# Shigangli/Ok-Topk

Hardware: NVIDIA H100
Metric: train_samples_per_sec_vgg16_oktopk_density0.001 (higher is better)
Workload: dtype fp32

## Files before the change

oktopk_b200/csrc/bindings.cpp:

```cpp
#include <pybind11/pybind11.h>
#include <pybind11/stl.h>
#include <cuda.h>
#include <cuda_runtime.h>

#include <unistd.h>

#include <algorithm>
#include <cstring>
#include <stdexcept>
#include <string>
#include <tuple>
#include <vector>

#include "oktopk.cuh"

namespace py = pybind11;
using namespace okt;

static void ck(cudaError_t e, const char* what) {
    if (e != cudaSuccess) throw std::runtime_error(std::string(what) + ": " + cudaGetErrorString(e));
}
template <class T> static T* P_(uint64_t p) { return reinterpret_cast<T*>(p); }
static cudaStream_t S_(uint64_t s) { return reinterpret_cast<cudaStream_t>(s); }

// ... 97 lines not shown
}
static uint64_t vmm_import(int fd) {
    auto imp = drv::sym<CUresult (*)(CUmemGenericAllocationHandle*, void*, CUmemAllocationHandleType)>("cuMemImportFromShareableHandle");
    CUmemGenericAllocationHandle h = 0;
    drv::ckd(imp(&h, reinterpret_cast<void*>(static_cast<uintptr_t>(fd)), CU_MEM_HANDLE_TYPE_POSIX_FILE_DESCRIPTOR), "cuMemImportFromShareableHandle");
    return (uint64_t)h;
}
static uint64_t vmm_map(uint64_t handle, size_t nbytes, int dev, size_t align) {
    auto reserve = drv::sym<CUresult (*)(CUdeviceptr*, size_t, size_t, CUdeviceptr, unsigned long long)>("cuMemAddressReserve");
    auto map = drv::sym<CUresult (*)(CUdeviceptr, size_t, size_t, CUmemGenericAllocationHandle, unsigned long long)>("cuMemMap");
    auto access = drv::sym<CUresult (*)(CUdeviceptr, size_t, const CUmemAccessDesc*, size_t)>("cuMemSetAccess");
    CUdeviceptr va = 0;
    drv::ckd(reserve(&va, nbytes, align, 0, 0), "cuMemAddressReserve");
    drv::ckd(map(va, nbytes, 0, (CUmemGenericAllocationHandle)handle, 0), "cuMemMap");
    CUmemAccessDesc ad;
    std::memset(&ad, 0, sizeof(ad));
    ad.location.type = CU_MEM_LOCATION_TYPE_DEVICE;
    ad.location.id = dev;
    ad.flags = CU_MEM_ACCESS_FLAGS_PROT_READWRITE;
    drv::ckd(access(va, nbytes, &ad, 1), "cuMemSetAccess");
    return (uint64_t)va;
}
static void vmm_unmap(uint64_t va, size_t nbytes) {
    auto unmap = drv::sym<CUresult (*)(CUdeviceptr, size_t)>("cuMemUnmap");
    auto afree = drv::sym<CUresult (*)(CUdeviceptr, size_t)>("cuMemAddressFree");
    unmap((CUdeviceptr)va, nbytes);
    afree((CUdeviceptr)va, nbytes);
}
static void vmm_release(uint64_t handle) {
    auto rel = drv::sym<CUresult (*)(CUmemGenericAllocationHandle)>("cuMemRelease");
    rel((CUmemGenericAllocationHandle)handle);
}
static py::tuple mc_create(size_t nbytes, int ndev) {
    auto create = drv::sym<CUresult (*)(CUmemGenericAllocationHandle*, const CUmulticastObjectProp*)>("cuMulticastCreate");
    auto exp = drv::sym<CUresult (*)(void*, CUmemGenericAllocationHandle, CUmemAllocationHandleType, unsigned long long)>("cuMemExportToShareableHandle");
    CUmulticastObjectProp mp;
    std::memset(&mp, 0, sizeof(mp));
    mp.numDevices = ndev; mp.size = nbytes; mp.handleTypes = CU_MEM_HANDLE_TYPE_POSIX_FILE_DESCRIPTOR;
    CUmemGenericAllocationHandle h = 0;
    drv::ckd(create(&h, &mp), "cuMulticastCreate");
    int fd = -1;
    drv::ckd(exp(&fd, h, CU_MEM_HANDLE_TYPE_POSIX_FILE_DESCRIPTOR, 0), "cuMemExportToShareableHandle(mc)");
    return py::make_tuple((uint64_t)h, fd);
}
static void mc_add_device(uint64_t mc, int dev) {
    auto add = drv::sym<CUresult (*)(CUmemGenericAllocationHandle, CUdevice)>("cuMulticastAddDevice");
    drv::ckd(add((CUmemGenericAllocationHandle)mc, dev), "cuMulticastAddDevice");
}
static void mc_bind(uint64_t mc, uint64_t mem, size_t nbytes) {
    auto bind = drv::sym<CUresult (*)(CUmemGenericAllocationHandle, size_t, CUmemGenericAllocationHandle, size_t, size_t, unsigned long long)>("cuMulticastBindMem");
    drv::ckd(bind((CUmemGenericAllocationHandle)mc, 0, (CUmemGenericAllocationHandle)mem, 0, nbytes, 0), "cuMulticastBindMem");
}

static size_t state_bytes() { return sizeof(OktState); }

static py::dict layout_info(int P, int n, int cap, int gcap) {
    SymmLayout L = make_layout(P, n, cap, gcap);
    py::dict d;
    d["total"] = L.total; d["rs_mbox"] = L.rs_mbox; d["rs_thr"] = L.rs_thr; d["ag_mbox"] = L.ag_mbox;
    d["cut_mbox"] = L.cut_mbox; d["cut_data"] = L.cut_data; d["send_idx"] = L.send_idx; d["send_val"] = L.send_val;
    d["gat_idx"] = L.gat_idx; d["gat_val"] = L.gat_val; d["cap"] = L.cap; d["gcap"] = L.gcap; d["scap"] = L.scap;
    d["done_mbox"] = L.done_mbox; d["tree_mbox"] = L.tree_mbox; d["scale_mbox"] = L.scale_mbox;
    d["chunk"] = kChunk; d["maxp"] = OKT_MAXP; d["threads"] = kThreads;
    return d;
}

static py::dict read_state(uint64_t st, int P, uint64_t stream) {
    static thread_local std::vector<char> host(offsetof(OktState, hist));
    ck(cudaMemcpyAsync(host.data(), P_<void>(st), host.size(), cudaMemcpyDeviceToHost, S_(stream)), "read_state");
    ck(cudaStreamSynchronize(S_(stream)), "read_state sync");
    const OktState* s = reinterpret_cast<const OktState*>(host.data());
    py::dict d;
    d["local_thr"] = s->local_thr; d["local_thr_used"] = s->local_thr_used; d["global_thr"] = s->global_thr;
    d["epoch"] = s->epoch;
    std::vector<int> e(s->edges, s->edges + P + 1);
    d["edges"] = e;
    d["local_count"] = s->stat_local_count; d["global_count"] = s->stat_global_count;
    d["recv_total"] = s->stat_recv_total; d["gather_total"] = s->stat_gather_total;
    d["overflow_send"] = s->stat_overflow_send; d["overflow_gather"] = s->stat_overflow_gather;
    d["redo"] = s->stat_redo; d["dense_fallback"] = s->stat_dense_fallback; d["pack_thr"] = s->pack_thr;
    d["cum_overflow_send"] = s->cum_overflow_send; d["cum_overflow_gather"] = s->cum_overflow_gather;
    d["cum_redo"] = s->cum_redo;
    d["fault"] = s->fault;
    auto us = [&](int a, int b) { return s->t_phase[b] >= s->t_phase[a] ? (double)(s->t_phase[b] - s->t_phase[a]) * 1e-3 : 0.0; };
    py::dict ph;
    ph["local"] = us(5, 0); ph["pack"] = us(0, 1); ph["wait_rs"] = us(1, 6); ph["reduce"] = us(6, 2); ph["gselect"] = us(2, 3);
    ph["wait_ag"] = us(3, 7); ph["final"] = us(7, 4); ph["total"] = us(5, 4);
    d["phase_us"] = ph;
    return d;
}

static py::list read_trace(uint64_t st, uint64_t stream) {
    std::vector<TraceRec> host(kTraceLen);
    ck(cudaMemcpyAsync(host.data(), reinterpret_cast<char*>(P_<OktState>(st)) + offsetof(OktState, trace),
                       sizeof(TraceRec) * kTraceLen, cudaMemcpyDeviceToHost, S_(stream)), "read_trace");
    ck(cudaStreamSynchronize(S_(stream)), "read_trace sync");
    py::list out;
    for (const TraceRec& t : host) {
        if (t.epoch == 0) continue;
        py::dict d;
        d["epoch"] = t.epoch; d["local_count"] = t.local_count; d["global_count"] = t.global_count;
        d["recv_total"] = t.recv_total; d["gather_total"] = t.gather_total; d["overflow_send"] = t.overflow_send;
        d["overflow_gather"] = t.overflow_gather; d["redo"] = t.redo; d["local_thr"] = t.local_thr;
        d["global_thr"] = t.global_thr; d["us_local"] = t.us_local; d["us_pack"] = t.us_pack;
        d["us_wait_rs"] = t.us_wait_rs; d["us_reduce"] = t.us_reduce; d["us_gselect"] = t.us_gselect;
        d["us_wait_ag"] = t.us_wait_ag; d["us_final"] = t.us_final; d["t_begin"] = t.t_begin;
        out.append(d);
    }
    return out;
}

static py::tuple host_flag_alloc() {
    int* h = nullptr;
    ck(cudaHostAlloc(reinterpret_cast<void**>(&h), sizeof(int) * 16, cudaHostAllocMapped), "cudaHostAlloc(flag)");
    for (int i = 0; i < 16; ++i) h[i] = 0;
    void* d = nullptr;
    ck(cudaHostGetDevicePointer(&d, h, 0), "cudaHostGetDevicePointer");
    return py::make_tuple((uint64_t)h, (uint64_t)d);
}
static void host_flag_free(uint64_t h) { if (h) cudaFreeHost(P_<void>(h)); }
static int host_flag_read(uint64_t h) { return h ? *reinterpret_cast<volatile int*>(h) : 0; }
static void host_flag_clear(uint64_t h) { if (h) *reinterpret_cast<volatile int*>(h) = 0; }

static void write_state(uint64_t st, float local_thr, float global_thr, const std::vector<int>& edges, uint64_t stream) {
    std::vector<char> host(offsetof(OktState, hist));
    ck(cudaMemcpyAsync(host.data(), P_<void>(st), host.size(), cudaMemcpyDeviceToHost, S_(stream)), "write_state rd");
    ck(cudaStreamSynchronize(S_(stream)), "write_state sync");
    OktState* s = reinterpret_cast<OktState*>(host.data());
    s->local_thr = local_thr;
    s->global_thr = global_thr;
    if (!edges.empty()) {
        if (edges.size() > OKT_MAXP + 1) throw std::runtime_error("too many region edges");
        for (size_t i = 0; i < edges.size(); ++i) s->edges[i] = edges[i];
    }
    ck(cudaMemcpyAsync(P_<void>(st), host.data(), host.size(), cudaMemcpyHostToDevice, S_(stream)), "write_state wr");
    ck(cudaStreamSynchronize(S_(stream)), "write_state sync2");
}

static void fill_peers(char** dst, const std::vector<uint64_t>& peers) {
    if (peers.size() > OKT_MAXP) throw std::runtime_error("world larger than OKT_MAXP");
    for (int i = 0; i < OKT_MAXP; ++i) dst[i] = nullptr;
    for (size_t i = 0; i < peers.size(); ++i) dst[i] = P_<char>(peers[i]);
}

static void oktopk_run(uint64_t g, uint64_t res, uint64_t st, const std::vector<uint64_t>& peers, int n, int rank,
                       int k, int cap, int gcap, py::dict o, int grid, uint64_t stream) {
    OktParams p;
    std::memset(&p, 0, sizeof(p));
    p.g = P_<float>(g); p.res = P_<float>(res); p.st = P_<OktState>(st);
    if (!o.contains("cand") || !o.contains("ccap")) throw std::runtime_error("oktopk_run: candidate scratch missing");
    p.cand = P_<int>(o["cand"].cast<uint64_t>()); p.ccap = o["ccap"].cast<int>();
    p.cand_mode = o.contains("cand_mode") ? o["cand_mode"].cast<int>() : 1;
    fill_peers(p.peers, peers);
    p.P = (int)peers.size(); p.rank = rank; p.n = n; p.k = k;
    p.L = make_layout(p.P, n, cap, gcap);
    auto geti = [&](const char* key, int dflt) { return o.contains(key) ? o[key].cast<int>() : dflt; };
    auto getf = [&](const char* key, double dflt) { return o.contains(key) ? o[key].cast<double>() : dflt; };
    for (int i = 0; i < OKT_MAXP; ++i) p.peer_g[i] = nullptr;
    if (o.contains("peer_g")) {
        auto pg = o["peer_g"].cast<std::vector<uint64_t>>();
        for (size_t i = 0; i < pg.size() && i < OKT_MAXP; ++i) p.peer_g[i] = P_<float>(pg[i]);
    }
    p.max_redo = geti("max_redo", 12);
    p.redo_factor = (float)getf("redo_factor", 1.5);
    p.dense_nnz_limit = geti("dense_nnz_limit", 0);
    p.host_fault = o.contains("host_fault") ? P_<int>(o["host_fault"].cast<uint64_t>()) : nullptr;
    p.skip = o.contains("skip") ? P_<const int>(o["skip"].cast<uint64_t>()) : nullptr;
    p.trace = geti("trace", 0);
    p.exact_local = geti("exact_local", 0);
    p.repartition = geti("repartition", 0);
    p.uniform_regions = geti("uniform_regions", 0);
    p.residual_mode = geti("residual_mode", RES_OKTOPK);
    p.global_mode = geti("global_mode", GLB_THRESHOLD);
    p.deterministic = geti("deterministic", 0);
    p.pull_tma = geti("pull_tma", 1);
    p.phase_begin = geti("phase_begin", 0);
    p.phase_end = geti("phase_end", PH_END);
    p.guard_loops = geti("guard_loops", 0);
    if (p.guard_loops > kGuardFineMax) p.guard_loops = kGuardFineMax;
    p.cap_limit = geti("cap_limit", 0);
    p.cap_rungs = geti("cap_rungs", 40);
    p.cap_factor = (float)getf("cap_factor", 1.19);
    p.guard_limit = geti("guard_limit", 0);
    p.guard_factor = (float)getf("guard_factor", 1.03);
    p.l_low_cnt = getf("l_low_cnt", 0.0); p.l_high_cnt = getf("l_high_cnt", 1e30);
    p.l_factor = (float)getf("l_factor", 1.012);
    p.g_low_cnt = getf("g_low_cnt", 0.0); p.g_high_cnt = getf("g_high_cnt", 1e30);
    p.g_inc = (float)getf("g_inc", 1.008); p.g_dec = (float)getf("g_dec", 1.008);
    p.prefilter = (float)getf("prefilter", 0.8);
    p.timeout_ns = (unsigned long long)(getf("timeout_s", 0.0) * 1e9);
    if (o.contains("srcs")) {
        auto t = o["srcs"].cast<std::tuple<std::vector<uint64_t>, std::vector<long long>, std::vector<long long>>>();
        const auto& ptr = std::get<0>(t);
        const auto& off = std::get<1>(t);
        const auto& len = std::get<2>(t);
        if (off.size() != ptr.size() || len.size() != ptr.size()) throw std::runtime_error("oktopk_run: srcs table size mismatch");
        if (ptr.size() > (size_t)kSrcSegMax) throw std::runtime_error("oktopk_run: more gradient sources than kSrcSegMax");
        long long end = 0;
        for (size_t i = 0; i < ptr.size(); ++i) {
            if (off[i] < end || (off[i] & 3) || len[i] <= 0 || off[i] + len[i] > n || (ptr[i] & 15))
                throw std::runtime_error("oktopk_run: gradient sources must be 16-byte aligned, in bucket order, "
                                         "non-overlapping, at offsets that are multiples of 4 elements");
            p.src[i] = P_<const float>(ptr[i]);
            p.src_off[i] = (int)off[i];
            p.src_len[i] = (int)len[i];
            end = off[i] + len[i];
        }
        p.nsrc = (int)ptr.size();
        p.zero_g = 0;
    } else {
        if (g & 15) throw std::runtime_error("oktopk_run: the bucket must be 16-byte aligned");
        p.src[0] = P_<const float>(g);
        p.src_off[0] = 0;
        p.src_len[0] = n;
        p.nsrc = 1;
        p.zero_g = 1;
    }
    if (o.contains("pack_ranges")) {
        auto rs = o["pack_ranges"].cast<std::vector<std::pair<long long, long long>>>();
        if (rs.size() > (size_t)kPackRangeMax) throw std::runtime_error("oktopk_run: more pack ranges than kPackRangeMax");
        long long end = 0;
        for (size_t i = 0; i < rs.size(); ++i) {
            const long long lo = rs[i].first, hi = rs[i].second;
            if (lo < end || hi < lo || (lo & 3) || (hi & 3) || hi > ((long long)n & ~3LL))
                throw std::runtime_error("oktopk_run: pack ranges must be ordered, disjoint, at multiples of 4 elements, "
                                         "inside the bucket's whole vectors");
            p.pk_lo[i] = (int)(lo >> 2);
            p.pk_hi[i] = (int)(hi >> 2);
            end = hi;
        }
        p.pk_mode = 1;
        p.pk_nr = (int)rs.size();
        if (geti("segment", 0)) {
            if (rs.empty() || p.zero_g || p.L.cap > 0 || p.residual_mode != RES_OKTOPK)
                throw std::runtime_error("oktopk_run: a segment launch takes ranges of an Ok-Topk bucket read from its "
// ... 67 lines not shown
static void land_grads(const std::vector<uint64_t>& srcs, const std::vector<long long>& offs, const std::vector<int>& numels,
                       uint64_t bucket, uint64_t stream) {
    const size_t T = srcs.size();
    if (offs.size() != T || numels.size() != T) throw std::runtime_error("land_grads: table size mismatch");
    constexpr int per = 8192;
    for (size_t b = 0; b < T; b += kLandMax) {
        LandParams lp;
        std::memset(&lp, 0, sizeof(lp));
        const int cnt = (int)std::min<size_t>(kLandMax, T - b);
        int blk = 0;
        for (int i = 0; i < cnt; ++i) {
            lp.src[i] = P_<const float>(srcs[b + i]);
            lp.dst_off[i] = offs[b + i];
            lp.numel[i] = numels[b + i];
            lp.blk_begin[i] = blk;
            blk += std::max(1, (numels[b + i] + per - 1) / per);
        }
        lp.blk_begin[cnt] = blk;
        lp.count = cnt;
        ck(launch_land(lp, P_<float>(bucket), S_(stream)), "land_grads");
    }
}

static void dense_run(const std::vector<uint64_t>& bufs, const std::vector<uint64_t>& flags, uint64_t epoch, int n,
                      int rank, int grid, uint64_t stream, uint64_t st, double timeout_s, uint64_t mc,
                      uint64_t host_fault, uint64_t skip) {
    DenseParams p;
    std::memset(&p, 0, sizeof(p));
    if (bufs.size() > OKT_MAXP || bufs.size() != flags.size()) throw std::runtime_error("bad peer tables");
    for (size_t i = 0; i < bufs.size(); ++i) { p.bufs[i] = P_<float>(bufs[i]); p.flags[i] = P_<uint64_t>(flags[i]); }
    p.epoch = P_<unsigned long long>(epoch);
    p.n = n; p.P = (int)bufs.size(); p.rank = rank; p.scale = 1.0f / (float)p.P;
    p.fault = st ? &P_<OktState>(st)->fault : nullptr;
    p.timeout_ns = (unsigned long long)(timeout_s * 1e9);
    p.mc = P_<float>(mc);
    p.host_fault = P_<int>(host_fault);
    p.skip = P_<const int>(skip);
    ck(launch_dense_allreduce(p, grid, S_(stream)), "dense allreduce launch");
}

static void kth_abs(uint64_t x, int n, int k, uint64_t st, uint64_t out, int grid, uint64_t stream) {
    ck(launch_kth_abs(P_<float>(x), n, k, P_<OktState>(st), P_<float>(out), grid, S_(stream)), "kth_abs launch");
}

static void fused_sgd(uint64_t p, uint64_t g, uint64_t mom, int n, double momentum, double dampening, double wd,
                      int nesterov, int first, int zero_grad, uint64_t stream, uint64_t scal_ptr, uint64_t fault_ptr,
                      uint64_t skip_ptr, uint64_t coef_ptr) {
    if (scal_ptr == 0) throw std::runtime_error("fused_sgd: scal_ptr must point at the group's device scalars");
    ck(launch_fused_sgd(P_<float>(p), P_<float>(g), P_<float>(mom), n, (float)momentum, (float)dampening, (float)wd,
                        nesterov, first, zero_grad, P_<float>(scal_ptr), P_<int>(fault_ptr), P_<int>(skip_ptr),
                        P_<const float>(coef_ptr), S_(stream)),
       "fused_sgd");
}
static SgdRanges sgd_ranges(const std::vector<std::pair<long long, long long>>& rs, int n, const char* what) {
    if ((int)rs.size() > kPackRangeMax)
        throw std::runtime_error(std::string(what) + ": more than " + std::to_string(kPackRangeMax) + " ranges");
    SgdRanges r;
    std::memset(&r, 0, sizeof(r));
    r.nr = (int)rs.size();
    for (int q = 0; q < r.nr; ++q) {
        const long long lo = rs[q].first, hi = rs[q].second;
        if (lo < 0 || hi < lo || lo % 4 || hi % 4 || hi > 4LL * (n / 4))
            throw std::runtime_error(std::string(what) + ": ranges must lie at multiples of 4 inside the slice's whole "
                                     "float4 vectors");
        r.lo[q] = (int)(lo / 4);
        r.hi[q] = (int)(hi / 4);
    }
    return r;
}
static void sgd_ahead(uint64_t p, uint64_t mom, uint64_t sp, uint64_t sm, int n,
                      const std::vector<std::pair<long long, long long>>& ranges, double momentum, double dampening,
                      double wd, int nesterov, int max_ctas, uint64_t stream, uint64_t scal_ptr) {
    if (scal_ptr == 0) throw std::runtime_error("sgd_ahead: scal_ptr must point at the group's device scalars");
    if (momentum != 0.0 && (mom == 0 || sm == 0)) throw std::runtime_error("sgd_ahead: momentum needs mom and sm");
    const SgdHyper h{(float)momentum, (float)dampening, (float)wd, nesterov, 0};
    ck(launch_sgd_ahead(P_<float>(p), P_<float>(mom), P_<float>(sp), P_<float>(sm), sgd_ranges(ranges, n, "sgd_ahead"),
                        h, max_ctas, P_<float>(scal_ptr), S_(stream)),
       "sgd_ahead");
}
static void fused_sgd_tail(uint64_t p, uint64_t g, uint64_t mom, uint64_t sp, uint64_t sm, int n,
                           const std::vector<std::pair<long long, long long>>& ahead,
                           const std::vector<std::pair<long long, long long>>& dense, double momentum, double dampening,
                           double wd, int nesterov, int first, int zero_grad, uint64_t stream, uint64_t scal_ptr,
                           uint64_t fault_ptr, uint64_t skip_ptr, uint64_t coef_ptr) {
    if (scal_ptr == 0) throw std::runtime_error("fused_sgd_tail: scal_ptr must point at the group's device scalars");
    if (momentum != 0.0 && (mom == 0 || sm == 0)) throw std::runtime_error("fused_sgd_tail: momentum needs mom and sm");
    const SgdHyper h{(float)momentum, (float)dampening, (float)wd, nesterov, first};
    ck(launch_fused_sgd_tail(P_<float>(p), P_<float>(g), P_<float>(mom), P_<const float>(sp), P_<const float>(sm), n,
                             sgd_ranges(ahead, n, "fused_sgd_tail"), sgd_ranges(dense, n, "fused_sgd_tail"), h,
                             zero_grad, P_<float>(scal_ptr), P_<int>(fault_ptr), P_<int>(skip_ptr),
                             P_<const float>(coef_ptr), S_(stream)),
       "fused_sgd_tail");
}
static void fused_bert_adam(uint64_t p, uint64_t g, uint64_t m, uint64_t v, int n, double b1, double b2, double eps,
                            double wd, int zero_grad, uint64_t stream, uint64_t scal_ptr, uint64_t fault_ptr,
                            uint64_t skip_ptr, uint64_t coef_ptr, uint64_t ends_ptr) {
    if (scal_ptr == 0) throw std::runtime_error("fused_bert_adam: scal_ptr must point at the group's device scalars");
    if (ends_ptr != 0 && coef_ptr == 0) throw std::runtime_error("fused_bert_adam: segment ends need the factors");
    const ClipRef clip{P_<const float>(coef_ptr), P_<const int>(ends_ptr)};
    ck(launch_fused_bert_adam(P_<float>(p), P_<float>(g), P_<float>(m), P_<float>(v), n, (float)b1, (float)b2,
                              (float)eps, (float)wd, zero_grad, P_<float>(scal_ptr), P_<int>(fault_ptr), P_<int>(skip_ptr),
                              clip, S_(stream)),
       "fused_bert_adam");
}
static void fused_adam(uint64_t p, uint64_t g, uint64_t m, uint64_t v, int n, double beta1, double beta2, double eps,
                       double wd, int decoupled, int zero_grad, uint64_t stream, uint64_t scal_ptr, uint64_t fault_ptr,
                       uint64_t skip_ptr, uint64_t coef_ptr) {
    if (scal_ptr == 0) throw std::runtime_error("fused_adam: scal_ptr must point at the group's device scalars");
    ck(launch_fused_adam(P_<float>(p), P_<float>(g), P_<float>(m), P_<float>(v), n, beta1, beta2, (float)eps, (float)wd,
                         decoupled, zero_grad, P_<float>(scal_ptr), P_<int>(fault_ptr), P_<int>(skip_ptr),
                         P_<const float>(coef_ptr), S_(stream)),
       "fused_adam");
}
static void fused_lamb(uint64_t p, uint64_t g, uint64_t m, uint64_t v, int n, double beta1, double beta2, double eps,
                       int nseg, uint64_t off, uint64_t len, uint64_t blk, uint64_t ends, int nblk, uint64_t part_w,
                       uint64_t part_u, uint64_t norm_w, uint64_t norm_u, uint64_t ratio, int zero_grad,
                       uint64_t stream, uint64_t scal_ptr, uint64_t fault_ptr, uint64_t skip_ptr, uint64_t coef_ptr) {
    if (scal_ptr == 0) throw std::runtime_error("fused_lamb: scal_ptr must point at the group's device scalars");
    if (nseg <= 0 || nblk < nseg || n < 0 || !off || !len || !blk || !ends || !part_w || !part_u || !norm_w || !norm_u ||
        !ratio)
        throw std::runtime_error("fused_lamb: bad segment table or buffers");
    if ((p | g | m | v) % 16 || (part_w | part_u) % 8)
        throw std::runtime_error("fused_lamb: p, g, m and v must be 16-byte aligned");
    const LambSegs t{P_<const int>(off), P_<const int>(len), P_<const int>(blk), P_<const int>(ends), nseg};
    ck(launch_fused_lamb(P_<float>(p), P_<float>(g), P_<float>(m), P_<float>(v), n, beta1, beta2, (float)eps, t, nblk,
                         P_<double>(part_w), P_<double>(part_u), P_<float>(norm_w), P_<float>(norm_u), P_<float>(ratio),
                         zero_grad, P_<float>(scal_ptr), P_<int>(fault_ptr), P_<int>(skip_ptr),
                         P_<const float>(coef_ptr), S_(stream)),
       "fused_lamb");
}
static Dtype dtype_arg(int dtype, const char* what) {
    if (dtype < 0 || dtype > 2) throw std::runtime_error(std::string(what) + ": dtype must be 0 (fp32), 1 (bf16) or 2 (fp16)");
    return static_cast<Dtype>(dtype);
}
static void bn_forward(uint64_t x, uint64_t y, uint64_t arg, uint64_t partial, uint64_t gamma, uint64_t beta, uint64_t cbias,
                       uint64_t save_mean, uint64_t save_invstd, uint64_t rmean, uint64_t rvar, uint64_t nbt, double momentum,
                       double eps, int relu, int M, int C, int W, int slot, int max_ctas, uint64_t stream, int dtype,
                       uint64_t res) {
    if (C % 4 != 0) throw std::runtime_error("bn_forward: channel count must be a multiple of 4");
    if (slot < 0) throw std::runtime_error("bn_forward: negative slot");
    if (res != 0 && (W != 0 || !relu)) throw std::runtime_error("bn_forward: a residual needs relu = 1 and no pool");
    ck(launch_bn_forward(P_<const void>(x), P_<void>(y), P_<unsigned char>(arg), P_<float>(partial), P_<const float>(gamma),
                         P_<const float>(beta), P_<const float>(cbias), P_<float>(save_mean), P_<float>(save_invstd),
                         P_<float>(rmean), P_<float>(rvar), P_<long long>(nbt), (float)momentum, (float)eps, relu, M, C, W, slot,
                         max_ctas, dtype_arg(dtype, "bn_forward"), S_(stream), P_<const void>(res)), "bn_forward");
}
static void bn_backward(uint64_t x, uint64_t dy, uint64_t arg, uint64_t dx, uint64_t partial, uint64_t gamma, uint64_t beta,
                        uint64_t save_mean, uint64_t save_invstd, uint64_t dgamma, uint64_t dbeta, int relu, int M, int C, int W,
                        int slot, int max_ctas, uint64_t stream, int dtype, uint64_t res, uint64_t dres) {
    if (slot < 0) throw std::runtime_error("bn_backward: negative slot");
    if ((res == 0) != (dres == 0)) throw std::runtime_error("bn_backward: res and dres go together");
    if (res != 0 && (W != 0 || !relu)) throw std::runtime_error("bn_backward: a residual needs relu = 1 and no pool");
    ck(launch_bn_backward(P_<const void>(x), P_<const void>(dy), P_<const unsigned char>(arg), P_<void>(dx), P_<float>(partial),
                          P_<const float>(gamma), P_<const float>(beta), P_<const float>(save_mean), P_<const float>(save_invstd),
                          P_<float>(dgamma), P_<float>(dbeta), relu, M, C, W, slot, max_ctas, dtype_arg(dtype, "bn_backward"),
                          S_(stream), P_<const void>(res), P_<void>(dres)), "bn_backward");
}
static void ln_check(const char* what, int R, int H, long long p_keep_thr, uint64_t seed, uint64_t mean, uint64_t rstd,
                     std::initializer_list<uint64_t> vec_ptrs) {
    if (R <= 0 || !ln_supported_h(H)) throw std::runtime_error(std::string(what) + ": needs R > 0 and H in 128, 256, ..., 1024");
    if (p_keep_thr < 0 || p_keep_thr > (1LL << 32)) throw std::runtime_error(std::string(what) + ": p_keep_thr out of range");
    if (p_keep_thr < (1LL << 32) && seed == 0) throw std::runtime_error(std::string(what) + ": dropout needs the seed");
    if (mean == 0 || rstd == 0) throw std::runtime_error(std::string(what) + ": mean and rstd are needed");
    for (uint64_t p : vec_ptrs)
        if (p == 0 || (p & 15)) throw std::runtime_error(std::string(what) + ": tensors must be non-null and 16-byte aligned");
}
static void ln_forward(uint64_t x, uint64_t a, uint64_t y, uint64_t gamma, uint64_t beta, uint64_t mean, uint64_t rstd,
                       uint64_t seed, int R, int H, long long p_keep_thr, double scale, double eps, int a_dtype,
                       uint64_t stream) {
    ln_check("ln_forward", R, H, p_keep_thr, seed, mean, rstd, {x, a, y, gamma, beta});
    ck(launch_ln_forward(P_<const float>(x), P_<const void>(a), P_<float>(y), P_<const float>(gamma), P_<const float>(beta),
                         P_<float>(mean), P_<float>(rstd), P_<const unsigned long long>(seed), R, H, p_keep_thr, (float)scale,
                         (float)eps, dtype_arg(a_dtype, "ln_forward"), S_(stream)), "ln_forward");
}
// ... 261 lines not shown
        t.nseg = (int)std::min<size_t>(kSrcSegMax, T - b);
        long long blk = 0;
        for (int i = 0; i < t.nseg; ++i) {
            const long long o = offs[b + i], l = lens[b + i];
            if (o < 0 || o % 4 || l < 0 || o + l > (1LL << 31) - 1)
                throw std::runtime_error("grad_sumsq: segments must lie at multiples of 4 inside an int32 range");
            t.off[i] = (int)o;
            t.len[i] = (int)l;
            t.blk_begin[i] = (int)blk;
            blk += std::max(1LL, (l + kSumsqChunk - 1) / kSumsqChunk);
        }
        t.blk_begin[t.nseg] = (int)blk;
        ck(launch_grad_sumsq(P_<const float>(g), t, out, S_(stream)), "grad_sumsq");
        out += blk;
    }
}
static void clip_coef(uint64_t partial, int np, uint64_t seg_blk, uint64_t seg_scal, int nseg, uint64_t scal,
                      double max_norm, uint64_t norm, uint64_t coef, uint64_t stream) {
    if (seg_blk != 0 && (seg_scal == 0 || scal == 0 || nseg <= 0))
        throw std::runtime_error("clip_coef: per-segment factors need seg_scal, scal and nseg");
    ck(launch_clip_coef(P_<const double>(partial), np, P_<const int>(seg_blk), P_<const int>(seg_scal), nseg,
                        P_<const float>(scal), (float)max_norm, P_<float>(norm), P_<float>(coef), S_(stream)),
       "clip_coef");
}

static void unscale_check(const std::vector<uint64_t>& srcs, const std::vector<long long>& lens, uint64_t ls, uint64_t sync,
                          uint64_t st, uint64_t host_fault, const std::vector<uint64_t>& peers, size_t mbox_off, int rank,
                          double timeout_s, uint64_t stream) {
    ScaleParams p;
    std::memset(&p, 0, sizeof(p));
    if (srcs.empty() || srcs.size() != lens.size()) throw std::runtime_error("unscale_check: bad source table");
    if (srcs.size() > (size_t)kSrcSegMax) throw std::runtime_error("unscale_check: more gradient sources than kSrcSegMax");
    if (peers.size() > OKT_MAXP) throw std::runtime_error("world larger than OKT_MAXP");
    int blk = 0;
    for (size_t i = 0; i < srcs.size(); ++i) {
        if ((srcs[i] & 15) || lens[i] <= 0 || lens[i] > (1LL << 31) - 1)
            throw std::runtime_error("unscale_check: sources must be 16-byte aligned and non-empty");
        p.src[i] = P_<float>(srcs[i]);
        p.len[i] = (int)lens[i];
        p.blk_begin[i] = blk;
        blk += (int)((lens[i] + kScalePerCta - 1) / kScalePerCta);
    }
    p.blk_begin[srcs.size()] = blk;
    p.nseg = (int)srcs.size();
    p.ls = P_<LossScaleDev>(ls);
    p.sync = P_<ScaleSync>(sync);
    p.fault = &P_<OktState>(st)->fault;
    p.host_fault = P_<int>(host_fault);
    for (size_t i = 0; i < peers.size(); ++i) p.peers[i] = P_<char>(peers[i]);
    p.mbox_off = mbox_off;
    p.P = (int)peers.size(); p.rank = rank;
    p.timeout_ns = (unsigned long long)(timeout_s * 1e9);
    ck(launch_unscale_check(p, S_(stream)), "unscale_check");
}

PYBIND11_MODULE(_C, m) {
    m.doc() = "oktopk_b200 native extension (sm_90a kernels + symmetric peer memory)";
    m.def("symm_alloc", &symm_alloc);
    m.def("symm_open", &symm_open);
    m.def("symm_close", &symm_close);
    m.def("symm_free", &symm_free);
    m.def("dev_alloc_zero", &dev_alloc_zero);
    m.def("dev_free", &dev_free);
    m.def("memset_async", &memset_async);
    m.def("can_access_peer", &can_access_peer);
    m.def("state_bytes", &state_bytes);
    m.def("layout_info", &layout_info);
    m.def("read_state", &read_state);
    m.def("write_state", &write_state);
    m.def("max_coop_grid", &okt_max_coop_grid);
    m.def("oktopk_run", &oktopk_run);
    m.def("gather_run", &gather_run);
    m.def("dense_run", &dense_run, py::arg("bufs"), py::arg("flags"), py::arg("epoch"), py::arg("n"), py::arg("rank"),
          py::arg("grid"), py::arg("stream"), py::arg("st") = 0, py::arg("timeout_s") = 0.0, py::arg("mc") = 0,
          py::arg("host_fault") = 0, py::arg("skip") = 0);
    m.def("gtopk_run", &gtopk_run);
    m.def("land_grads", &land_grads);
    m.def("read_trace", &read_trace);
    m.def("host_flag_alloc", &host_flag_alloc);
    m.def("host_flag_free", &host_flag_free);
    m.def("host_flag_read", &host_flag_read);
    m.def("host_flag_clear", &host_flag_clear);
    m.def("fault_ptr", [](uint64_t st) { return (uint64_t)&P_<OktState>(st)->fault; });
    m.def("gather_max_coop_grid", &gather_max_coop_grid);
    m.def("gtopk_max_coop_grid", &gtopk_max_coop_grid);
    m.def("vmm_probe", &vmm_probe);
    m.def("vmm_create", &vmm_create);
    m.def("vmm_import", &vmm_import);
    m.def("vmm_map", &vmm_map);
    m.def("vmm_unmap", &vmm_unmap);
    m.def("vmm_release", &vmm_release);
    m.def("mc_create", &mc_create);
    m.def("mc_add_device", &mc_add_device);
    m.def("mc_bind", &mc_bind);
    m.def("close_fd", [](int fd) { if (fd >= 0) ::close(fd); });
    m.def("clear_fault", [](uint64_t st, uint64_t stream) {
        ck(cudaMemsetAsync(&P_<OktState>(st)->fault, 0, sizeof(int), S_(stream)), "clear_fault");
    });
    m.def("kth_abs", &kth_abs);
    m.def("fused_sgd", &fused_sgd, py::arg("p"), py::arg("g"), py::arg("mom"), py::arg("n"), py::arg("momentum"),
          py::arg("dampening"), py::arg("wd"), py::arg("nesterov"), py::arg("first"), py::arg("zero_grad"),
          py::arg("stream"), py::arg("scal_ptr"), py::arg("fault_ptr") = 0, py::arg("skip_ptr") = 0,
          py::arg("coef_ptr") = 0);
    m.def("sgd_ahead", &sgd_ahead, py::arg("p"), py::arg("mom"), py::arg("sp"), py::arg("sm"), py::arg("n"),
          py::arg("ranges"), py::arg("momentum"), py::arg("dampening"), py::arg("wd"), py::arg("nesterov"),
          py::arg("max_ctas"), py::arg("stream"), py::arg("scal_ptr"));
    m.def("fused_sgd_tail", &fused_sgd_tail, py::arg("p"), py::arg("g"), py::arg("mom"), py::arg("sp"), py::arg("sm"),
          py::arg("n"), py::arg("ahead"), py::arg("dense"), py::arg("momentum"), py::arg("dampening"), py::arg("wd"),
          py::arg("nesterov"), py::arg("first"), py::arg("zero_grad"), py::arg("stream"), py::arg("scal_ptr"),
          py::arg("fault_ptr") = 0, py::arg("skip_ptr") = 0, py::arg("coef_ptr") = 0);
    m.def("fused_bert_adam", &fused_bert_adam, py::arg("p"), py::arg("g"), py::arg("m"), py::arg("v"), py::arg("n"),
          py::arg("b1"), py::arg("b2"), py::arg("eps"), py::arg("wd"), py::arg("zero_grad"), py::arg("stream"),
          py::arg("scal_ptr"), py::arg("fault_ptr") = 0, py::arg("skip_ptr") = 0, py::arg("coef_ptr") = 0,
          py::arg("ends_ptr") = 0);
    m.def("fused_adam", &fused_adam, py::arg("p"), py::arg("g"), py::arg("m"), py::arg("v"), py::arg("n"),
          py::arg("beta1"), py::arg("beta2"), py::arg("eps"), py::arg("wd"), py::arg("decoupled"), py::arg("zero_grad"),
          py::arg("stream"), py::arg("scal_ptr"), py::arg("fault_ptr") = 0, py::arg("skip_ptr") = 0,
          py::arg("coef_ptr") = 0);
    m.def("fused_lamb", &fused_lamb, py::arg("p"), py::arg("g"), py::arg("m"), py::arg("v"), py::arg("n"),
          py::arg("beta1"), py::arg("beta2"), py::arg("eps"), py::arg("nseg"), py::arg("off"), py::arg("len"),
          py::arg("blk"), py::arg("ends"), py::arg("nblk"), py::arg("part_w"), py::arg("part_u"), py::arg("norm_w"),
          py::arg("norm_u"), py::arg("ratio"), py::arg("zero_grad"), py::arg("stream"), py::arg("scal_ptr"),
          py::arg("fault_ptr") = 0, py::arg("skip_ptr") = 0, py::arg("coef_ptr") = 0);
    m.def("momentum_correct", &momentum_correct);
    m.def("grad_sumsq", &grad_sumsq, py::arg("g"), py::arg("offs"), py::arg("lens"), py::arg("partial"),
          py::arg("stream"));
    m.def("clip_coef", &clip_coef, py::arg("partial"), py::arg("np"), py::arg("seg_blk"), py::arg("seg_scal"),
          py::arg("nseg"), py::arg("scal"), py::arg("max_norm"), py::arg("norm"), py::arg("coef"), py::arg("stream"));
    m.def("unscale_check", &unscale_check);
    m.def("scale_update", [](uint64_t ls, double growth, double backoff, int interval, uint64_t stream) {
        ck(launch_scale_update(P_<LossScaleDev>(ls), growth, backoff, interval, S_(stream)), "scale_update");
    });
    m.def("adam_scalars", [](uint64_t ls, uint64_t hyper, uint64_t scal, int groups, uint64_t stream, int lamb) {
        ck(launch_adam_scalars(P_<const LossScaleDev>(ls), P_<const double>(hyper), P_<float>(scal), groups, lamb,
                               S_(stream)),
           "adam_scalars");
    }, py::arg("ls"), py::arg("hyper"), py::arg("scal"), py::arg("groups"), py::arg("stream"), py::arg("lamb") = 0);
    m.def("carry_residual", [](uint64_t g, uint64_t res, int n, uint64_t skip, uint64_t stream) {
        ck(launch_carry_residual(P_<float>(g), P_<float>(res), n, P_<const int>(skip), S_(stream)), "carry_residual");
    });
    m.attr("LOSS_SCALE_BYTES") = sizeof(LossScaleDev);
    m.attr("SCALE_SYNC_BYTES") = sizeof(ScaleSync);
    m.attr("VERDICT_OFFSET") = offsetof(ScaleSync, verdict);
    m.def("maxpool2_fwd", &maxpool2_fwd);
    m.def("maxpool2_bwd", &maxpool2_bwd);
    m.def("bn_forward", &bn_forward, py::arg("x"), py::arg("y"), py::arg("arg"), py::arg("partial"), py::arg("gamma"),
          py::arg("beta"), py::arg("cbias"), py::arg("save_mean"), py::arg("save_invstd"), py::arg("rmean"), py::arg("rvar"),
          py::arg("nbt"), py::arg("momentum"), py::arg("eps"), py::arg("relu"), py::arg("M"), py::arg("C"), py::arg("W"),
          py::arg("slot"), py::arg("max_ctas"), py::arg("stream"), py::arg("dtype"), py::arg("res") = 0);
    m.def("bn_backward", &bn_backward, py::arg("x"), py::arg("dy"), py::arg("arg"), py::arg("dx"), py::arg("partial"),
          py::arg("gamma"), py::arg("beta"), py::arg("save_mean"), py::arg("save_invstd"), py::arg("dgamma"), py::arg("dbeta"),
          py::arg("relu"), py::arg("M"), py::arg("C"), py::arg("W"), py::arg("slot"), py::arg("max_ctas"), py::arg("stream"),
          py::arg("dtype"), py::arg("res") = 0, py::arg("dres") = 0);
    m.def("bn_tile_rows", &bn_tile_rows);
    m.def("bn_sliced", &bn_sliced, py::arg("M"), py::arg("C"), py::arg("W"));
    m.def("ln_forward", &ln_forward, py::arg("x"), py::arg("a"), py::arg("y"), py::arg("gamma"), py::arg("beta"),
          py::arg("mean"), py::arg("rstd"), py::arg("seed"), py::arg("R"), py::arg("H"), py::arg("p_keep_thr"),
          py::arg("scale"), py::arg("eps"), py::arg("a_dtype"), py::arg("stream"));
    m.def("ln_backward", &ln_backward, py::arg("x"), py::arg("a"), py::arg("dy"), py::arg("gamma"), py::arg("mean"),
          py::arg("rstd"), py::arg("seed"), py::arg("dx"), py::arg("da"), py::arg("partial"), py::arg("dgamma"),
          py::arg("dbeta"), py::arg("R"), py::arg("H"), py::arg("p_keep_thr"), py::arg("scale"), py::arg("a_dtype"),
          py::arg("stream"));
    m.def("ln_bwd_grid", &ln_bwd_grid);
    m.def("ln_supported_h", &ln_supported_h);
    m.def("emb_forward", &emb_forward, py::arg("ids"), py::arg("tt"), py::arg("word"), py::arg("pos"), py::arg("typ"),
          py::arg("gamma"), py::arg("beta"), py::arg("y"), py::arg("stats"), py::arg("ovf"), py::arg("seed"), py::arg("R"),
          py::arg("S"), py::arg("H"), py::arg("nv"), py::arg("np"), py::arg("nt"), py::arg("p_keep_thr"), py::arg("scale"),
          py::arg("eps"), py::arg("stream"));
    m.def("emb_backward", &emb_backward, py::arg("ids"), py::arg("tt"), py::arg("word"), py::arg("pos"), py::arg("typ"),
          py::arg("gamma"), py::arg("stats"), py::arg("dy"), py::arg("seed"), py::arg("de"), py::arg("partial"), py::arg("dgamma"), py::arg("dbeta"), py::arg("dword"), py::arg("dpos"), py::arg("dtyp"),
          py::arg("R"), py::arg("S"), py::arg("H"), py::arg("nv"), py::arg("np"), py::arg("nt"), py::arg("p_keep_thr"),
          py::arg("scale"), py::arg("stream"));
    m.def("emb_supported", &emb_supported);
    m.def("attn_forward", &attn_forward, py::arg("qkv"), py::arg("mask"), py::arg("seed"), py::arg("out"), py::arg("lse"),
          py::arg("B"), py::arg("S"), py::arg("H"), py::arg("p_keep_thr"), py::arg("scale"), py::arg("dtype"),
          py::arg("stream"));
    m.def("attn_backward", &attn_backward, py::arg("qkv"), py::arg("out"), py::arg("dout"), py::arg("mask"), py::arg("seed"),
          py::arg("lse"), py::arg("delta"), py::arg("dqkv"), py::arg("B"), py::arg("S"), py::arg("H"), py::arg("p_keep_thr"),
          py::arg("scale"), py::arg("dtype"), py::arg("stream"));
    m.def("attn_supported", &attn_supported);
    m.def("xent_forward", &xent_forward, py::arg("x"), py::arg("t"), py::arg("lse"), py::arg("rowloss"), py::arg("loss"),
          py::arg("R"), py::arg("V"), py::arg("ignore_index"), py::arg("dtype"), py::arg("stream"));
    m.def("xent_backward", &xent_backward, py::arg("x"), py::arg("t"), py::arg("lse"), py::arg("g"), py::arg("dx"),
          py::arg("R"), py::arg("V"), py::arg("ignore_index"), py::arg("dtype"), py::arg("stream"));
    m.def("ctc_forward", &ctc_forward, py::arg("x"), py::arg("t"), py::arg("t64"), py::arg("tn"), py::arg("ln"),
          py::arg("ws"), py::arg("loss"), py::arg("T"), py::arg("N"), py::arg("C"), py::arg("nt"), py::arg("dtype"),
          py::arg("stream"));
    m.def("ctc_backward", &ctc_backward, py::arg("x"), py::arg("t"), py::arg("t64"), py::arg("tn"), py::arg("ln"),
          py::arg("ws"), py::arg("ab"), py::arg("g"), py::arg("dx"), py::arg("T"), py::arg("N"), py::arg("C"), py::arg("nt"),
          py::arg("dtype"), py::arg("stream"));
    m.def("ctc_supported", &ctc_supported);
    m.def("frame_bn_forward", &frame_bn_forward, py::arg("conv"), py::arg("x"), py::arg("len"), py::arg("gamma"),
          py::arg("beta"), py::arg("y"), py::arg("mean"), py::arg("rstd"), py::arg("rmean"), py::arg("rvar"),
// ... 43 lines not shown
```

oktopk_b200/csrc/oktopk.cu:

```cuda
#include "devlib.cuh"

namespace okt {

__device__ __forceinline__ int region_of(const int* s_edges, int P, int i) {
    int d = 0;
#pragma unroll 1
    for (int r = 1; r < P; ++r) d += (i >= s_edges[r]) ? 1 : 0;
    return d;
}

struct SrcSeg { const float* src; int off, len; };

__device__ __forceinline__ int seg_find(const SrcSeg* s, int ns, int e) {
    int lo = 0, hi = ns - 1, r = -1;
    while (lo <= hi) {
        const int mid = (lo + hi) >> 1;
        if (s[mid].off <= e) { r = mid; lo = mid + 1; } else { hi = mid - 1; }
    }
    return r;
}

__device__ __forceinline__ float grad_at(const SrcSeg* s, int ns, int i) {
    const int q = seg_find(s, ns, i);
    return (q >= 0 && i - s[q].off < s[q].len) ? s[q].src[i - s[q].off] : 0.f;
// ... 200 lines not shown
                const int lo_d = sel.edges[d], hi_d = sel.edges[d + 1];
                mine = 0u;
#pragma unroll
                for (int u = 0; u < kPackTile; ++u) {
#pragma unroll
                    for (int c = 0; c < 4; ++c) {
                        const int i = 4 * (base + u * kThreads + tid) + c;
                        const bool pd = ((mybits >> (u * 4 + c)) & 1u) && i >= lo_d && i < hi_d;
                        md[u * 4 + c] = __ballot_sync(0xffffffffu, pd);
                        cnt += __popc(md[u * 4 + c]);
                        if (pd) mine |= 1u << (u * 4 + c);
                    }
                }
            }
            if (cnt == 0) continue;
            int run = 0;
            if (lane == 0) run = atomicAdd(&st->send_cursor[d], cnt);
            run = __shfl_sync(0xffffffffu, run, 0);
            const int scap_d = sel.soff[d + 1] - sel.soff[d];
            int* sidx = sel.sidx + sel.soff[d];
            float* sval = sel.sval + sel.soff[d];
            const int off_d = sel.edges[d];
            const unsigned lt = (1u << lane) - 1u;
#pragma unroll
            for (int u = 0; u < kPackTile; ++u) {
                const float xs[4] = {a[u].x, a[u].y, a[u].z, a[u].w};
#pragma unroll
                for (int c = 0; c < 4; ++c) {
                    const int q = u * 4 + c;
                    if ((mine >> q) & 1u) {
                        const int pos = run + __popc(md[q] & lt);
                        const int i = 4 * (base + u * kThreads + tid) + c;
                        if (pos < scap_d) {
                            sidx[pos] = i - off_d;
                            sval[pos] = xs[c];
                            if (p.residual_mode != RES_OKTOPK) p.res[i] = 0.f;
                        } else {
                            dropped++;
                        }
                    }
                    run += __popc(md[q]);
                }
            }
        }
    }
    return nmine;
}

__global__ void __launch_bounds__(kThreads, kCtasPerSm) oktopk_fused_kernel(const OktParams p) {
    __shared__ uint32_t s_hist[kHistBins];
    __shared__ int s_w[kWarps + 1];
    __shared__ int s_edges[OKT_MAXP + 1];
    __shared__ int s_cnt[OKT_MAXP];
    __shared__ float s_thr[OKT_MAXP];
    __shared__ int s_misc[OKT_MAXP * 2 + 4];
    __shared__ int s_soff[OKT_MAXP + 1];
    __shared__ float s_lthr[kGuardMax];
    __shared__ int s_lcnt[kGuardMax];
    __shared__ ChunkSrc s_srcs[OKT_MAXP];
    __shared__ float s_sthr[OKT_MAXP];
    __shared__ Seg s_segs[OKT_MAXP];
    __shared__ __align__(128) PullSmem s_pull;
    __shared__ __align__(8) uint64_t s_pk_bar[kPackStages];
    __shared__ __align__(8) uint64_t s_pk_empty[kPackStages];
    __shared__ __align__(8) uint64_t s_sc_bar[kScanStages];
    __shared__ SrcSeg s_src[kSrcSegMax];
    __shared__ int s_tail_v[kSrcSegMax], s_tail_q[kSrcSegMax];
    __shared__ int s_ntail;
    __shared__ int s_rlo[kPackRangeMax], s_rhi[kPackRangeMax], s_rfirst[kPackRangeMax + 1];
    extern __shared__ __align__(128) float4 dyn_pk[];

    if (verdict_set(p.skip)) return;
    OktState* st = p.st;
    const int tid = threadIdx.x, lane = tid & 31, warp = tid >> 5;
    const int gtid = blockIdx.x * kThreads + tid;
    const int gthreads = gridDim.x * kThreads;
    const int P = p.P, rank = p.rank, n = p.n;
    char* me = p.peers[rank];
    const uint32_t epoch = st->epoch + 1u;
    const int par = epoch & 1u;
    const float thr_in = st->local_thr;
    const bool exact_local = p.exact_local || thr_in == 0.f;
    const bool two_pass = exact_local || p.repartition;
    uint32_t pipe_it = 0;

    for (int b = tid; b < kHistBins; b += kThreads) s_hist[b] = 0;
    if (blockIdx.x == 0 && tid == 0) st->t_phase[5] = globaltimer_ns();
    const SpinGuard sg_rs{&st->fault, p.timeout_ns, FAULT_RS_TIMEOUT, p.host_fault};
    const SpinGuard sg_ag{&st->fault, p.timeout_ns, FAULT_AG_TIMEOUT, p.host_fault};
    const SpinGuard sg_cut{&st->fault, p.timeout_ns, FAULT_CUT_TIMEOUT, p.host_fault};
    const SpinGuard sg_done{&st->fault, p.timeout_ns, FAULT_DONE_TIMEOUT, p.host_fault};
    if (tid == 0) {
        mbar_init(&s_pull.bar[0], 1);
        mbar_init(&s_pull.bar[1], 1);
        for (int q = 0; q < kPackStages; ++q) { mbar_init(&s_pk_bar[q], 1); mbar_init(&s_pk_empty[q], kWarps); }
        for (int q = 0; q < kScanStages; ++q) mbar_init(&s_sc_bar[q], 1);
        mbar_fence_init();
    }
    const int n4 = n >> 2;
    const int nsrc = p.nsrc;
    load_src_table(p, s_src, s_tail_v, s_tail_q, &s_ntail);
    const int ntail = s_ntail;
    const int whole[2] = {0, n4};
    const bool ranged = p.pk_mode && !two_pass;
    const TileMap tmap = tile_map_build(ranged ? p.pk_nr : 1, ranged ? p.pk_lo : whole, ranged ? p.pk_hi : whole + 1,
                                        s_rlo, s_rhi, s_rfirst);

    float4* r4 = reinterpret_cast<float4*>(p.res);

    if (p.phase_begin <= PH_LOCAL && PH_LOCAL < p.phase_end && two_pass) {
        const float thr0 = thr_in;
        const LadderCfg lcl = ladder_cfg(p, !exact_local);
        ladder_build(s_lthr, s_lcnt, lcl, thr0);

        auto visit = [&](float x) {
            if (exact_local) {
                hist_add(s_hist, x, 0, 0u);
            } else {
                float ax = fabsf(x);
                if (ax > thr0) atomicAdd(&s_lcnt[ladder_rung(s_lthr, lcl.n_total, ax)], 1);
            }
        };
        const float cut = (exact_local && thr0 > 0.f) ? thr0 * p.prefilter : -1.f;
        const bool prefilter = cut > 0.f;
        constexpr int kLocTile = 4;
        for (int base = blockIdx.x * kThreads * kLocTile; base < n4; base += gridDim.x * kThreads * kLocTile) {
            float4 a[kLocTile], r[kLocTile];
            bool in[kLocTile];
#pragma unroll
            for (int u = 0; u < kLocTile; ++u) {
                const int v = base + u * kThreads + tid;
                in[u] = v < n4;
                if (in[u]) { a[u] = grad4_at(s_src, nsrc, v); r[u] = ld_stream_f4(r4 + v); }
                else { a[u] = make_float4(0.f, 0.f, 0.f, 0.f); r[u] = a[u]; }
            }
#pragma unroll
            for (int u = 0; u < kLocTile; ++u) {
                const int v = base + u * kThreads + tid;
                a[u].x += r[u].x; a[u].y += r[u].y; a[u].z += r[u].z; a[u].w += r[u].w;
                if (in[u]) st_stream_f4(r4 + v, a[u]);
                const float xs[4] = {a[u].x, a[u].y, a[u].z, a[u].w};
                if (!prefilter) {
                    if (in[u]) { visit(xs[0]); visit(xs[1]); visit(xs[2]); visit(xs[3]); }
                    continue;
                }
                unsigned bits = 0u;
                int tot = 0;
#pragma unroll
                for (int c = 0; c < 4; ++c) {
                    const bool pd = in[u] && fabsf(xs[c]) > cut;
                    if (pd) bits |= 1u << c;
                    tot += __popc(__ballot_sync(0xffffffffu, pd));
                }
                if (tot == 0) continue;
                int run = 0;
                if (lane == 0) run = atomicAdd(&st->cand_cursor, tot);
                run = __shfl_sync(0xffffffffu, run, 0);
#pragma unroll
                for (int c = 0; c < 4; ++c) {
                    const bool pd = (bits >> c) & 1u;
                    const unsigned m = __ballot_sync(0xffffffffu, pd);
                    if (pd) {
                        const int pos = run + __popc(m & ((1u << lane) - 1u));
                        if (pos < p.ccap) p.cand[pos] = 4 * v + c;
                    }
                    run += __popc(m);
// ... 165 lines not shown
            auto emit = [&](int i, float x, bool inrange) {
                const float ax = fabsf(x);
                const bool pred = inrange && ax > thr_sel;
                unsigned todo = __ballot_sync(0xffffffffu, pred);
                if (todo == 0) return;
                int d = 0;
                if (pred) {
                    d = region_of(s_edges, P, i);
                    atomicAdd(&s_lcnt[lc.n_total > 1 ? ladder_rung(s_lthr, lc.n_total, ax) : 0], 1);
                }
                while (todo) {
                    const int leader = __ffs(todo) - 1;
                    const int dl = __shfl_sync(0xffffffffu, d, leader);
                    const bool mine = pred && d == dl;
                    const unsigned m = __ballot_sync(0xffffffffu, mine);
                    int base = 0;
                    if (lane == leader) base = atomicAdd(&st->send_cursor[dl], __popc(m));
                    base = __shfl_sync(0xffffffffu, base, leader);
                    if (mine) {
                        const int pos = base + __popc(m & ((1u << lane) - 1u));
                        if (pos < s_soff[dl + 1] - s_soff[dl]) {
                            my_sidx[s_soff[dl] + pos] = i - s_edges[dl];
                            my_sval[s_soff[dl] + pos] = x;
                            if (p.residual_mode != RES_OKTOPK) p.res[i] = 0.f;
                        } else {
                            dropped++;
                        }
                    }
                    todo &= ~m;
                }
            };

            const PackSrc src{s_src, nsrc, s_tail_v, s_tail_q, ntail};
            const PackSel sel{thr_sel, lc, s_lthr, s_lcnt, s_edges, s_soff, my_sidx, my_sval, P};
            ring_it += pack_stream<kPackStages>(p, tmap, ring, ring_it, res_only, attempt == 0 && p.zero_g, src, sel, dropped);
            if (blockIdx.x == 0 && warp == 0 && (n & 3)) {
                int i = n4 * 4 + lane;
                bool in = i < n;
                float a = 0.f;
                if (in) {
                    a = res_only ? p.res[i] : (grad_at(s_src, nsrc, i) + p.res[i]);
                    if (!res_only) p.res[i] = a;
                    if (p.zero_g) p.g[i] = 0.f;
                }
                emit(i, a, in);
            }
            if (p.residual_mode == RES_LOCAL_GE && blockIdx.x == 0 && (n & 3)) {
                for (int i = n4 * 4 + tid; i < n; i += kThreads) {
                    float x = p.res[i];
                    if (x != 0.f && fabsf(x) == thr_sel && atomicAdd(&st->tie_cursor, 1) < (int)__ldcg(&st->sel_krem))
                        p.res[i] = 0.f;
                }
            }
            ladder_flush(st, s_lcnt);
            if (!can_redo) break;
            grid_sync(&st->bar);
            bool over = false;
            for (int d = 0; d < P; ++d) over = over || (__ldcg(&st->send_cursor[d]) > s_soff[d + 1] - s_soff[d]);
            if (!over || attempt >= p.max_redo) break;
            grid_sync(&st->bar);
            if (blockIdx.x == 0 && tid == 0) {
                for (int d = 0; d < P; ++d) st->send_cursor[d] = 0;
                for (int q = 0; q < kGuardMax; ++q) st->guard_counts[q] = 0;
                st->cum_redo += 1ULL;
            }
            thr_sel = fmaxf(thr_sel, 1e-30f) * redo_f;
            redo_f = fminf(redo_f * redo_f, 1e6f);
            ++attempt;
            grid_sync(&st->bar);
        }
        {
            int dsum = warp_sum(dropped);
            if (lane == 0 && dsum) atomicAdd(&st->cum_overflow_send, (unsigned long long)dsum);
        }
        const bool publisher = can_redo ? (blockIdx.x == 0) : last_cta_ticket(&st->tick[0]);
        if (publisher) {
            if (tid == 0) {
                int cnt;
                const float t = ladder_pick(st, ladder_cfg(p, !two_pass), thr_sel, p.guard_limit, p.cap_limit, &cnt);
                st->local_thr_used = t;
                st->pack_thr = thr_sel;
                st->stat_local_count = cnt;
                st->tie_cursor = 0;
                float nt = t;
                if ((double)cnt < p.l_low_cnt) nt = t / p.l_factor;
                else if ((double)cnt > p.l_high_cnt) nt = t * p.l_factor;
                st->local_thr = nt;
                s_thr[0] = t;
                __threadfence();
            }
            __syncthreads();
            if (tid < P) {
                const int c = min(__ldcg(&st->send_cursor[tid]), s_soff[tid + 1] - s_soff[tid]);
                st_relaxed_sys_u32(reinterpret_cast<uint32_t*>(rs_thr(p.peers[tid], p.L, par, rank)), __float_as_uint(s_thr[0]));
                st_release_sys_u64(rs_mbox(p.peers[tid], p.L, par, rank), make_mail(epoch, (uint32_t)c));
            }
            __syncthreads();
        }
        stamp(1);
    }

    if (p.phase_begin <= PH_REDUCE && PH_REDUCE < p.phase_end) {
        if (tid < P) {
            s_cnt[tid] = (int)wait_mailbox(rs_mbox(me, p.L, par, tid), epoch, sg_rs);
            s_thr[tid] = __uint_as_float(ld_relaxed_sys_u32(reinterpret_cast<uint32_t*>(rs_thr(me, p.L, par, tid))));
        }
        __syncthreads();
        stamp(6);
        const int off_me = s_edges[rank];
        const int len_me = s_edges[rank + 1] - off_me;
        float* greg = p.g + off_me;
        int pulled = 0;
        auto add = [&](int s_local, int idx, float val, const float* thr_of) {
            const bool ok = fabsf(val) > thr_of[s_local] && (unsigned)idx < (unsigned)len_me;
            if (p.cand_mode) {
                float old = 1.f;
                if (ok) old = atomicAdd(greg + idx, val);
                const bool first = ok && old == 0.f;
                const int pos = warp_append_active(&st->cand_cursor, first);
                if (first && pos < p.ccap) p.cand[pos] = idx;
            } else if (ok) {
                red_add_f32(greg + idx, val);
            }
            pulled++;
        };
        const int my_soff = s_soff[rank];
        if (!p.deterministic) {
            if (tid < P) {
                const int s = (rank + tid) % P;
                s_srcs[tid].idx = send_idx_base(p.peers[s], p.L) + my_soff;
                s_srcs[tid].val = send_val_base(p.peers[s], p.L) + my_soff;
                s_srcs[tid].count = s_cnt[s];
                s_sthr[tid] = s_thr[s];
            }
            __syncthreads();
            pull_chunks(s_srcs, P, p.pull_tma != 0, &s_pull, pipe_it,
                        [&](int sl, int idx, float val) { add(sl, idx, val, s_sthr); });
        } else {
            for (int s = 0; s < P; ++s) {
                ChunkSrc src{send_idx_base(p.peers[s], p.L) + my_soff, send_val_base(p.peers[s], p.L) + my_soff, s_cnt[s]};
                float thr1 = s_thr[s];
                pull_chunks(&src, 1, p.pull_tma != 0, &s_pull, pipe_it,
                            [&](int, int idx, float val) { add(0, idx, val, &thr1); });
                grid_sync(&st->bar);
            }
        }
        int psum = warp_sum(pulled);
        if (lane == 0 && psum) atomicAdd(&st->stat_recv_total, psum);
        if (PH_REDUCE + 1 < p.phase_end) grid_sync(&st->bar);
        stamp(2);
    }

    if (p.phase_begin <= PH_GSELECT && PH_GSELECT < p.phase_end) {
        const float gthr = st->global_thr;
        const int lo = s_edges[rank], hi = s_edges[rank + 1];
        const int gcap = p.L.gcap;
        int* gi = gat_idx(me, p.L, par);
        float* gv = gat_val(me, p.L, par);
        const bool keep_in_place = p.global_mode == GLB_ALL_NONZERO;
        int dropped = 0;
        if (p.cand_mode) {
            const int ncand = min(*reinterpret_cast<volatile int*>(&st->cand_cursor), p.ccap);
            const int ncr = (ncand + 31) / 32 * 32;
            for (int c = gtid; c < ncr; c += gthreads) {
                const bool in = c < ncand;
                const int i = in ? __ldcg(p.cand + c) : 0;
// ... 71 lines not shown
                        run += __popc(m);
                    }
                    if (!keep_in_place) {
                        if ((nzbits >> (u * 4)) & 0xfu)
                            *reinterpret_cast<float4*>(p.g + first + 4 * (q0 + u * kThreads + tid)) = make_float4(0.f, 0.f, 0.f, 0.f);
                    } else if ((lostbits >> (u * 4)) & 0xfu) {
#pragma unroll
                        for (int c = 0; c < 4; ++c)
                            if ((lostbits >> (u * 4 + c)) & 1u) p.g[first + 4 * (q0 + u * kThreads + tid) + c] = 0.f;
                    }
                }
            });
        }
        int dsum = warp_sum(dropped);
        if (lane == 0 && dsum) atomicAdd(&st->cum_overflow_gather, (unsigned long long)dsum);
        stamp(3);
        if (last_cta_ticket(&st->tick[1])) {
            if (tid == 0) s_misc[0] = min(__ldcg(&st->gather_cursor), p.L.gcap);
            __syncthreads();
            if (tid < P) st_release_sys_u64(ag_mbox(p.peers[tid], p.L, par, rank), make_mail(epoch, (uint32_t)s_misc[0]));
            __syncthreads();
        }
    }

    if (p.phase_begin <= PH_FINAL && PH_FINAL < p.phase_end) {
        if (tid < P) s_cnt[tid] = (int)wait_mailbox(ag_mbox(me, p.L, par, tid), epoch, sg_ag);
        __syncthreads();
        stamp(7);
        int T = 0;
        for (int s = 0; s < P; ++s) T += s_cnt[s];
        const float fP = (float)P;
        const bool dense_path = p.global_mode == GLB_ALL_NONZERO && p.dense_nnz_limit > 0 && T >= p.dense_nnz_limit &&
                                P > 1 && p.peer_g[0] != nullptr;
        int kept_cnt = 0;
        if (dense_path) {
            const float inv = 1.f / fP;
            for (int t = 1; t < P; ++t) {
                const int s = (rank + t) % P;
                const int lo_s = s_edges[s], hi_s = s_edges[s + 1];
                const float* src = p.peer_g[s];
                const int first = min(hi_s, (lo_s + 3) & ~3), last = max(first, hi_s & ~3);
                for (int i = lo_s + gtid; i < first; i += gthreads) p.g[i] = ld_peer_f32(src + i) * inv;
                for (int i = last + gtid; i < hi_s; i += gthreads) p.g[i] = ld_peer_f32(src + i) * inv;
                const int nv = (last - first) >> 2;
                const int4* s4 = reinterpret_cast<const int4*>(src + first);
                float4* d4 = reinterpret_cast<float4*>(p.g + first);
                for (int v = gtid; v < nv; v += gthreads) {
                    const int4 r = ld_peer_i4(s4 + v);
                    st_stream_f4(d4 + v, make_float4(__int_as_float(r.x) * inv, __int_as_float(r.y) * inv,
                                                     __int_as_float(r.z) * inv, __int_as_float(r.w) * inv));
                }
            }
            grid_sync(&st->bar);
            if (blockIdx.x == 0 && tid < P) st_release_sys_u64(done_mbox(p.peers[tid], p.L, par, rank), make_mail(epoch, 1u));
            if (tid < P) wait_mailbox(done_mbox(me, p.L, par, tid), epoch, sg_done);
            __syncthreads();
            const int lo = s_edges[rank], hi = s_edges[rank + 1];
            for (int i = lo + gtid; i < hi; i += gthreads) p.g[i] = __ldcg(p.g + i) * inv;
            if (blockIdx.x == 0 && tid == 0) { st->stat_dense_fallback = 1; st->stat_global_count = T; }
        } else {
            float gsel = 0.f;
            if (p.global_mode == GLB_EXACT_TOPK) {
                if (tid < P) { s_segs[tid].ptr = gat_val(p.peers[tid], p.L, par); s_segs[tid].count = s_cnt[tid]; s_segs[tid].idx = nullptr; }
                __syncthreads();
                const uint32_t kk = (uint32_t)min(T, p.k);
                gsel = (kk > 0) ? grid_kth_abs(s_segs, P, true, kk, st, s_hist, s_w, 0) : 0.f;
                if (blockIdx.x == 0 && tid == 0) st->global_thr = gsel;
            } else if (p.global_mode == GLB_THRESHOLD && blockIdx.x == 0 && tid == 0) {
                float gt = st->global_thr;
                if ((double)T < p.g_low_cnt) gt = gt / p.g_inc;
                else if ((double)T > p.g_high_cnt) gt = gt * p.g_dec;
                st->global_thr = gt;
            }
            const float thr_used = st->local_thr_used;
            if (tid < P) {
                const int s = (rank + tid) % P;
                s_srcs[tid].idx = gat_idx(p.peers[s], p.L, par);
                s_srcs[tid].val = gat_val(p.peers[s], p.L, par);
                s_srcs[tid].count = s_cnt[s];
            }
            __syncthreads();
            const bool exact = p.global_mode == GLB_EXACT_TOPK;
            pull_chunks(s_srcs, P, p.pull_tma != 0, &s_pull, pipe_it, [&](int sl, int idx, float val) {
                if ((unsigned)idx >= (unsigned)n) return;
                bool keep = exact ? (fabsf(val) >= gsel) : true;
                if (!keep) return;
                kept_cnt++;
                p.g[idx] = val / fP;
                if (p.residual_mode == RES_OKTOPK) {
                    float r = p.res[idx];
                    if (fabsf(r) > thr_used) p.res[idx] = 0.f;
                }
            });
            int ksum = warp_sum(kept_cnt);
            if (lane == 0 && ksum) atomicAdd(&st->stat_global_count, ksum);
        }
        if (last_cta_ticket(&st->tick[2]) && tid == 0) {
            const unsigned long long t_end = globaltimer_ns();
            st->epoch = epoch;
            st->t_phase[4] = t_end;
            st->stat_gather_total = T;
            for (int d = 0; d < P; ++d) st->send_cursor[d] = 0;
            st->gather_cursor = 0;
            st->cand_cursor = 0;
            const unsigned long long os = *reinterpret_cast<volatile unsigned long long*>(&st->cum_overflow_send);
            const unsigned long long og = *reinterpret_cast<volatile unsigned long long*>(&st->cum_overflow_gather);
            const unsigned long long rd = *reinterpret_cast<volatile unsigned long long*>(&st->cum_redo);
            st->stat_overflow_send = (int)min(os - st->snap_overflow_send, 0x7fffffffULL);
            st->stat_overflow_gather = (int)min(og - st->snap_overflow_gather, 0x7fffffffULL);
            st->stat_redo = (int)(rd - st->snap_redo);
            st->snap_overflow_send = os; st->snap_overflow_gather = og; st->snap_redo = rd;
            TraceRec& tr = st->trace[epoch % kTraceLen];
            auto us = [&](int a, int b) {
                const unsigned long long ta = *reinterpret_cast<volatile unsigned long long*>(&st->t_phase[a]);
                const unsigned long long tb = *reinterpret_cast<volatile unsigned long long*>(&st->t_phase[b]);
                return tb >= ta ? (float)(tb - ta) * 1e-3f : 0.f;
            };
            tr.epoch = epoch;
            tr.local_count = st->stat_local_count;
            tr.global_count = *reinterpret_cast<volatile int*>(&st->stat_global_count);
            tr.recv_total = *reinterpret_cast<volatile int*>(&st->stat_recv_total);
            tr.gather_total = T;
            tr.overflow_send = st->stat_overflow_send;
            tr.overflow_gather = st->stat_overflow_gather;
            tr.redo = st->stat_redo;
            tr.local_thr = st->local_thr_used;
            tr.global_thr = st->global_thr;
            tr.us_local = us(5, 0); tr.us_pack = us(0, 1); tr.us_wait_rs = us(1, 6); tr.us_reduce = us(6, 2);
            tr.us_gselect = us(2, 3); tr.us_wait_ag = us(3, 7); tr.us_final = us(7, 4);
            tr.t_begin = st->t_phase[5];
        }
    }
}

__global__ void __launch_bounds__(kThreads) oktopk_segment_kernel(const OktParams p) {
    __shared__ int s_edges[OKT_MAXP + 1];
    __shared__ int s_soff[OKT_MAXP + 1];
    __shared__ float s_lthr[kGuardMax];
    __shared__ int s_lcnt[kGuardMax];
    __shared__ __align__(8) uint64_t s_full[kSegStages];
    __shared__ __align__(8) uint64_t s_empty[kSegStages];
    __shared__ SrcSeg s_src[kSrcSegMax];
    __shared__ int s_tail_v[kSrcSegMax], s_tail_q[kSrcSegMax];
    __shared__ int s_ntail;
    __shared__ int s_rlo[kPackRangeMax], s_rhi[kPackRangeMax], s_rfirst[kPackRangeMax + 1];
    extern __shared__ __align__(128) float4 dyn_seg[];

    if (verdict_set(p.skip)) return;
    OktState* st = p.st;
    const float thr = st->local_thr;
    if (thr == 0.f) return;
    const int tid = threadIdx.x, P = p.P;
    if (tid == 0) {
        for (int q = 0; q < kSegStages; ++q) { mbar_init(&s_full[q], 1); mbar_init(&s_empty[q], kWarps); }
        mbar_fence_init();
    }
    if (tid <= P) s_edges[tid] = st->edges[tid];
    load_src_table(p, s_src, s_tail_v, s_tail_q, &s_ntail);
    if (tid <= P) s_soff[tid] = (tid < P) ? slot_off(p.L, s_edges, tid) : slot_off(p.L, s_edges, P);
    const TileMap tmap = tile_map_build(p.pk_nr, p.pk_lo, p.pk_hi, s_rlo, s_rhi, s_rfirst);
    const LadderCfg lc = ladder_cfg(p, true);
    ladder_build(s_lthr, s_lcnt, lc, thr);
    char* me = p.peers[p.rank];
    const PackRing ring{dyn_seg, dyn_seg + kSegStages * kTileV, s_full, s_empty};
    const PackSrc src{s_src, p.nsrc, s_tail_v, s_tail_q, s_ntail};
    const PackSel sel{thr, lc, s_lthr, s_lcnt, s_edges, s_soff, send_idx_base(me, p.L), send_val_base(me, p.L), P};
    int dropped = 0;
    pack_stream<kSegStages>(p, tmap, ring, 0, false, false, src, sel, dropped);
// ... 61 lines not shown
```

oktopk_b200/csrc/oktopk.cuh:

```cuda
#pragma once
#include <cuda_runtime.h>
#include <stdint.h>
#include <stddef.h>

#ifndef OKT_MAXP
#define OKT_MAXP 16
#endif

namespace okt {

constexpr int kThreads = 512;
constexpr int kWarps = kThreads / 32;
constexpr int kChunk = 1024;
constexpr int kHistBins = 2048;
constexpr int kMaxWarpsTotal = 16384;
constexpr int kGuardMax = 64;
constexpr int kGuardFineMax = 15;
constexpr int kCtasPerSm = 1;
constexpr int kPackTile = 2;
constexpr int kPackStages = 4;
constexpr int kPackSmemBytes = kPackStages * 2 * kPackTile * kThreads * 16;
constexpr int kScanStages = 2 * kPackStages;
constexpr int kStrideGridMax = 132 * 8;

constexpr int kTraceLen = 256;
struct TraceRec {
    uint32_t epoch;
    int local_count, global_count, recv_total, gather_total, overflow_send, overflow_gather, redo;
    float local_thr, global_thr;
    float us_local, us_pack, us_wait_rs, us_reduce, us_gselect, us_wait_ag, us_final;
    unsigned long long t_begin;
};

struct OktState {
    unsigned long long bar;
    unsigned int tick[4];
    float local_thr;
    float local_thr_used;
    float global_thr;
    uint32_t epoch;
    int edges[OKT_MAXP + 1];
    int send_cursor[OKT_MAXP];
    int gather_cursor;
    int cand_cursor;
    int guard_counts[kGuardMax];
    uint32_t sel_prefix;
    uint32_t sel_krem;
    int tie_cursor;
    int cuts[OKT_MAXP];
    int stat_local_count;
    int stat_global_count;
    int stat_recv_total;
    int stat_gather_total;
    int stat_overflow_send;
    int stat_overflow_gather;
    int stat_redo;
    int stat_dense_fallback;
    int stat_mode;
    int fault;
    float pack_thr;
    unsigned long long cum_overflow_send;
    unsigned long long cum_overflow_gather;
    unsigned long long cum_redo;
    unsigned long long snap_overflow_send;
    unsigned long long snap_overflow_gather;
    unsigned long long snap_redo;
    unsigned long long t_phase[8];
    double gs_sum, gs_sumsq;
    double clip_sumsq;
    uint32_t hist[kHistBins];
    int wcounts[kMaxWarpsTotal];
    TraceRec trace[kTraceLen];
};

struct SymmLayout {
    size_t rs_mbox;
    size_t rs_thr;
    size_t ag_mbox;
    size_t cut_mbox;
    size_t cut_data;
    size_t done_mbox;
    size_t tree_mbox;
    size_t scale_mbox;
    size_t send_idx;
    size_t send_val;
    size_t gat_idx;
    size_t gat_val;
    size_t total;
    int cap;
    int scap;
    int gcap;
};

inline size_t align_up(size_t x, size_t a) { return (x + a - 1) / a * a; }

inline SymmLayout make_layout(int P, int n, int cap, int gcap) {
    SymmLayout L;
    size_t o = 0;
    L.rs_mbox = o;  o += sizeof(uint64_t) * 2 * OKT_MAXP;
    L.rs_thr = o;   o += sizeof(float) * 2 * OKT_MAXP;
    L.ag_mbox = o;  o += sizeof(uint64_t) * 2 * OKT_MAXP;
    L.cut_mbox = o; o += sizeof(uint64_t) * 2 * OKT_MAXP;
    L.cut_data = o; o += sizeof(int) * 2 * OKT_MAXP * OKT_MAXP;
    L.done_mbox = o; o += sizeof(uint64_t) * 2 * OKT_MAXP;
    L.tree_mbox = o; o += sizeof(uint64_t) * 2 * OKT_MAXP;
    L.scale_mbox = o; o += sizeof(uint64_t) * 2 * OKT_MAXP;
    o = align_up(o, 1024);
    const size_t scap = cap > 0 ? (size_t)P * cap : align_up((size_t)n, 4) + 4 * (size_t)OKT_MAXP + 1024;
    L.send_idx = o; o += sizeof(int) * scap;   o = align_up(o, 1024);
    L.send_val = o; o += sizeof(float) * scap; o = align_up(o, 1024);
    L.gat_idx = o;  o += sizeof(int) * 2 * (size_t)gcap;      o = align_up(o, 1024);
    L.gat_val = o;  o += sizeof(float) * 2 * (size_t)gcap;    o = align_up(o, 1024);
    L.total = o;
    L.cap = cap;
    L.scap = (int)scap;
    L.gcap = gcap;
    return L;
}

enum Phase : int {
    PH_LOCAL = 0,
    PH_PACK = 1,
    PH_PUBLISH_RS = 2,
    PH_REDUCE = 3,
    PH_GSELECT = 4,
    PH_PUBLISH_AG = 5,
    PH_FINAL = 6,
    PH_END = 7
};

enum ResidualMode : int { RES_OKTOPK = 0, RES_LOCAL_GT = 1, RES_LOCAL_GE = 2 };
enum GlobalMode : int { GLB_THRESHOLD = 0, GLB_EXACT_TOPK = 1, GLB_ALL_NONZERO = 2 };

constexpr int kSrcSegMax = 160;
constexpr int kPackRangeMax = 32;
constexpr int kSegStages = 2;
constexpr int kSegTiles = 4;

struct OktParams {
    float* g;
    float* res;
    OktState* st;
    int* cand;
    int ccap;
    int cand_mode;
    float prefilter;
    char* peers[OKT_MAXP];
    float* peer_g[OKT_MAXP];
    SymmLayout L;
    int n, P, rank, k;
    int exact_local, repartition, uniform_regions;
    int residual_mode, global_mode;
    int deterministic, pull_tma;
    int phase_begin, phase_end;
    int guard_loops, guard_limit;
    float guard_factor;
    int cap_limit, cap_rungs;
    float cap_factor;
    double l_low_cnt, l_high_cnt;
    float l_factor;
    double g_low_cnt, g_high_cnt;
    float g_inc, g_dec;
    unsigned long long timeout_ns;
    int max_redo;
    float redo_factor;
    int dense_nnz_limit;
    int* host_fault;
    const int* skip;
    int trace;
    int zero_g;
    int nsrc;
    int src_off[kSrcSegMax];
    int src_len[kSrcSegMax];
    const float* src[kSrcSegMax];
    int pk_mode, pk_nr;
    int pk_lo[kPackRangeMax];
    int pk_hi[kPackRangeMax];
};
static_assert(sizeof(OktParams) <= 4096, "OktParams must fit the 4 KB kernel-parameter limit");

enum GatherSelect : int { GS_THRESHOLD_REUSE = 0, GS_GAUSSIAN = 1, GS_EXACT_TOPK = 2 };

struct GatherParams {
    float* g;
    float* res;
    OktState* st;
    char* peers[OKT_MAXP];
    SymmLayout L;
    int n, P, rank, k;
    int select_mode;
    int exact_now;
    int gauss_mode;
    int gauss_loops;
    float gauss_factor;
    float density;
    int pull_tma;
    unsigned long long timeout_ns;
    int reselect;
    float clip_max_norm;
    unsigned* bitmap;
    int* cand;
    int ccap;
    int* host_fault;
    const int* skip;
};

struct TreeParams {
    float* g;
    float* res;
    OktState* st;
    char* peers[OKT_MAXP];
    SymmLayout L;
    int n, P, rank, k;
    int pull_tma;
    unsigned long long timeout_ns;
    float clip_max_norm;
    unsigned* bitmap;
    int* cand;
    int ccap;
    int* sel_idx;
    float* sel_val;
    int selcap;
    int* host_fault;
    const int* skip;
};

struct DenseParams {
    float* bufs[OKT_MAXP];
    uint64_t* flags[OKT_MAXP];
    unsigned long long* epoch;
    int n, P, rank;
    float scale;
    int* fault;
    unsigned long long timeout_ns;
    float* mc;
    int* host_fault;
    const int* skip;
};

int okt_max_coop_grid(int device);
cudaError_t launch_oktopk(const OktParams& p, int grid, cudaStream_t stream);
cudaError_t launch_oktopk_segment(const OktParams& p, int max_ctas, cudaStream_t stream);
cudaError_t launch_gather_scheme(const GatherParams& p, int grid, cudaStream_t stream);
cudaError_t launch_gtopk(const TreeParams& p, int grid, cudaStream_t stream);
int gtopk_max_coop_grid(int device);
int gather_max_coop_grid(int device);
cudaError_t launch_dense_allreduce(const DenseParams& p, int grid, cudaStream_t stream);
cudaError_t launch_kth_abs(const float* x, int n, int k, OktState* st, float* out_thr, int grid, cudaStream_t stream);
constexpr int kSumsqChunk = 16384;
struct SumsqSegs {
    int nseg;
    int off[kSrcSegMax];
    int len[kSrcSegMax];
    int blk_begin[kSrcSegMax + 1];
};
static_assert(sizeof(SumsqSegs) <= 4096, "SumsqSegs must fit the 4 KB kernel-parameter limit");
cudaError_t launch_grad_sumsq(const float* g, const SumsqSegs& t, double* partial, cudaStream_t stream);
cudaError_t launch_clip_coef(const double* partial, int np, const int* seg_blk, const int* seg_scal, int nseg,
                             const float* scal, float max_norm, float* norm, float* coef, cudaStream_t stream);
struct ClipRef {
    const float* coef;
    const int* ends;
};
cudaError_t launch_fused_sgd(float* p, float* g, float* mom, int n, float momentum, float dampening, float weight_decay,
                             int nesterov, int first_step, int zero_grad, const float* scal, const int* fault,
                             const int* skip, const float* coef, cudaStream_t stream);
struct SgdRanges {
    int nr;
    int lo[kPackRangeMax];
    int hi[kPackRangeMax];
};
struct SgdHyper {
    float momentum, dampening, wd;
    int nesterov, first;
};
cudaError_t launch_sgd_ahead(float* p, float* mom, float* sp, float* sm, const SgdRanges& r, const SgdHyper& h,
                             int max_ctas, const float* scal, cudaStream_t stream);
cudaError_t launch_fused_sgd_tail(float* p, float* g, float* mom, const float* sp, const float* sm, int n,
                                  const SgdRanges& ahead, const SgdRanges& dense, const SgdHyper& h, int zero_grad,
                                  const float* scal, const int* fault, const int* skip, const float* coef,
                                  cudaStream_t stream);
cudaError_t launch_fused_bert_adam(float* p, float* g, float* m, float* v, int n, float b1, float b2, float eps,
                                   float weight_decay, int zero_grad, const float* scal, const int* fault,
                                   const int* skip, const ClipRef& clip, cudaStream_t stream);
cudaError_t launch_fused_adam(float* p, float* g, float* m, float* v, int n, double beta1, double beta2, float eps,
                              float weight_decay, int decoupled, int zero_grad, const float* scal, const int* fault,
                              const int* skip, const float* coef, cudaStream_t stream);
struct LambSegs {
    const int* off;
    const int* len;
    const int* blk;
    const int* ends;
    int nseg;
};
struct LambHyper {
    float b1, omb1, b2, omb2, eps;
};
cudaError_t launch_fused_lamb(float* p, float* g, float* m, float* v, int n, double beta1, double beta2, float eps,
                              const LambSegs& t, int nblk, double* part_w, double* part_u, float* norm_w,
                              float* norm_u, float* ratio, int zero_grad, const float* scal, const int* fault,
                              const int* skip, const float* coef, cudaStream_t stream);

struct LossScaleDev {
    float scale;
    float inv_scale;
    int growth_tracker;
    int found_inf;
    long long skipped;
    long long adam_step;
};
struct ScaleSync {
    int flag;
    unsigned int ticket;
    unsigned int epoch;
    int verdict;
};
constexpr int kScaleThreads = 256;
constexpr int kScalePerCta = 8192;
struct ScaleParams {
    LossScaleDev* ls;
    ScaleSync* sync;
    int* fault;
    int* host_fault;
    char* peers[OKT_MAXP];
    size_t mbox_off;
    int P, rank;
    unsigned long long timeout_ns;
    int nseg;
    int len[kSrcSegMax];
    int blk_begin[kSrcSegMax + 1];
    float* src[kSrcSegMax];
};
static_assert(sizeof(ScaleParams) <= 4096, "ScaleParams must fit the 4 KB kernel-parameter limit");
cudaError_t launch_unscale_check(const ScaleParams& p, cudaStream_t stream);
cudaError_t launch_scale_update(LossScaleDev* ls, double growth_factor, double backoff_factor, int growth_interval,
                                cudaStream_t stream);
cudaError_t launch_adam_scalars(const LossScaleDev* ls, const double* hyper, float* scal, int groups, int lamb,
                                cudaStream_t stream);
cudaError_t launch_carry_residual(float* g, float* res, int n, const int* skip, cudaStream_t stream);
constexpr int kLandMax = 96;
struct LandParams {
    const float* src[kLandMax];
    long long dst_off[kLandMax];
    int numel[kLandMax];
    int blk_begin[kLandMax + 1];
    int count;
};
cudaError_t launch_land(const LandParams& lp, float* bucket, cudaStream_t stream);
enum class Dtype : int { kF32 = 0, kBF16 = 1, kF16 = 2 };
int bn_tile_rows(int M, int C);
bool bn_sliced(int M, int C, int W);
cudaError_t launch_bn_forward(const void* x, void* y, unsigned char* arg, float* partial, const float* gamma, const float* beta,
                              const float* cbias, float* save_mean, float* save_invstd, float* rmean, float* rvar, long long* nbt,
                              float momentum, float eps, int relu, int M, int C, int W, int slot, int max_ctas, Dtype dtype,
                              cudaStream_t stream, const void* res = nullptr);
cudaError_t launch_bn_backward(const void* x, const void* dy, const unsigned char* arg, void* dx, float* partial,
                               const float* gamma, const float* beta, const float* save_mean, const float* save_invstd,
                               float* dgamma, float* dbeta, int relu, int M, int C, int W, int slot, int max_ctas, Dtype dtype,
                               cudaStream_t stream, const void* res = nullptr, void* dres = nullptr);
cudaError_t launch_maxpool2_fwd(const float* x, float* y, unsigned char* arg, int N, int H, int W, int C, cudaStream_t stream);
cudaError_t launch_maxpool2_bwd(const float* dy, const unsigned char* arg, float* dx, int N, int H, int W, int C,
                                cudaStream_t stream);
bool ln_supported_h(int H);
int ln_bwd_grid(int R);
// ... 73 lines not shown
```

oktopk_b200/csrc/optim.cu:

```cuda
#include "common.cuh"
#include "oktopk.cuh"

namespace okt {

constexpr int kOptThreads = 256;

struct ClipCursor {
    const float* coef;
    const int* ends;
    int t;
    float f;
    __device__ __forceinline__ explicit ClipCursor(const ClipRef& c)
        : coef(c.coef), ends(c.ends), t(0), f(c.coef != nullptr ? c.coef[0] : 1.f) {}
    __device__ __forceinline__ float at(int vec) {
        if (ends != nullptr && vec >= __ldg(ends + t)) {
            do ++t; while (vec >= __ldg(ends + t));
            f = coef[t];
        }
        return f;
    }
};

__device__ __forceinline__ void scale4(float4& gw, float c) {
    gw.x = __fmul_rn(gw.x, c); gw.y = __fmul_rn(gw.y, c); gw.z = __fmul_rn(gw.z, c); gw.w = __fmul_rn(gw.w, c);
}

template <int kScal, int kState, typename Upd>
__device__ __forceinline__ void update_pass(float* __restrict__ p, float* __restrict__ g, float* __restrict__ m,
                                            float* __restrict__ v, int n, bool load, bool store, int zero_grad,
                                            const float* __restrict__ scal, const int* __restrict__ fault,
                                            const int* __restrict__ skip, const ClipRef clip, Upd upd) {
    if (fault != nullptr && *reinterpret_cast<const volatile int*>(fault) != 0) return;
    const int n4 = n >> 2;
    float4* p4 = reinterpret_cast<float4*>(p);
    float4* g4 = reinterpret_cast<float4*>(g);
    float4* m4 = reinterpret_cast<float4*>(m);
    float4* v4 = reinterpret_cast<float4*>(v);
    const float4 zero = make_float4(0.f, 0.f, 0.f, 0.f);
    if (verdict_set(skip)) {
        if (!zero_grad) return;
        for (int i = blockIdx.x * kOptThreads + threadIdx.x; i < n4; i += gridDim.x * kOptThreads) {
            const float4 gw = ld_stream_f4(g4 + i);
            if (gw.x != 0.f || gw.y != 0.f || gw.z != 0.f || gw.w != 0.f) g4[i] = zero;
        }
        if (blockIdx.x == 0)
            for (int i = n4 * 4 + threadIdx.x; i < n; i += kOptThreads) g[i] = 0.f;
        return;
    }
    float s[kScal];
#pragma unroll
    for (int j = 0; j < kScal; ++j) s[j] = scal[j];
    ClipCursor cc(clip);
    for (int i = blockIdx.x * kOptThreads + threadIdx.x; i < n4; i += gridDim.x * kOptThreads) {
        float4 pw = p4[i], gw = ld_stream_f4(g4 + i), mw = zero, vw = zero;
        const bool dirty = gw.x != 0.f || gw.y != 0.f || gw.z != 0.f || gw.w != 0.f;
        if (clip.coef != nullptr) scale4(gw, cc.at(i));
        if (load) {
            mw = m4[i];
            if (kState == 2) vw = v4[i];
        }
        upd(s, pw.x, gw.x, mw.x, vw.x); upd(s, pw.y, gw.y, mw.y, vw.y);
        upd(s, pw.z, gw.z, mw.z, vw.z); upd(s, pw.w, gw.w, mw.w, vw.w);
        p4[i] = pw;
        if (store) {
            m4[i] = mw;
            if (kState == 2) v4[i] = vw;
        }
        if (zero_grad && dirty) g4[i] = zero;
    }
    if (blockIdx.x == 0)
        for (int i = n4 * 4 + threadIdx.x; i < n; i += kOptThreads) {
            float pw = p[i], gw = g[i], mw = 0.f, vw = 0.f;
            if (clip.coef != nullptr) gw = __fmul_rn(gw, cc.at(i >> 2));
            if (load) {
                mw = m[i];
                if (kState == 2) vw = v[i];
            }
            upd(s, pw, gw, mw, vw);
            p[i] = pw;
            if (store) {
                m[i] = mw;
                if (kState == 2) v[i] = vw;
            }
            if (zero_grad) g[i] = 0.f;
        }
}

__device__ __forceinline__ void sgd_update(const SgdHyper& h, float lr, float& pw, float gw, float& mw) {
    const float damp = h.first ? 0.f : h.dampening;
    float d = __fmaf_rn(h.wd, pw, gw);
    if (h.momentum != 0.f) {
        mw = h.first ? d : __fmaf_rn(1.f - damp, d, __fmul_rn(h.momentum, mw));
        d = h.nesterov ? __fmaf_rn(h.momentum, mw, d) : mw;
    }
    pw = __fmaf_rn(-lr, d, pw);
}

__device__ __forceinline__ void sgd_update4(const SgdHyper& h, float lr, float4& pw, const float4& gw, float4& mw) {
    sgd_update(h, lr, pw.x, gw.x, mw.x); sgd_update(h, lr, pw.y, gw.y, mw.y);
    sgd_update(h, lr, pw.z, gw.z, mw.z); sgd_update(h, lr, pw.w, gw.w, mw.w);
}

__global__ void __launch_bounds__(kOptThreads) fused_sgd_kernel(float* __restrict__ p, float* __restrict__ g,
                                                                 float* __restrict__ mom, int n, const SgdHyper h,
                                                                 int zero_grad, const float* __restrict__ scal,
                                                                 const int* __restrict__ fault,
                                                                 const int* __restrict__ skip,
                                                                 const float* __restrict__ coef) {
    update_pass<1, 1>(p, g, mom, nullptr, n, h.momentum != 0.f && !h.first, h.momentum != 0.f, zero_grad, scal, fault,
                      skip, ClipRef{coef, nullptr},
                      [=](const float* s, float& pw, float gw, float& mw, float&) { sgd_update(h, s[0], pw, gw, mw); });
}

constexpr int kAheadUnroll = 4;

__device__ __forceinline__ void st_evict_f4(float4* p, const float4& v) {
    asm volatile("st.global.cs.v4.f32 [%0], {%1,%2,%3,%4};" ::"l"(p), "f"(v.x), "f"(v.y), "f"(v.z), "f"(v.w) : "memory");
}

__global__ void __launch_bounds__(kOptThreads) sgd_ahead_kernel(float* __restrict__ p, float* __restrict__ mom,
                                                                 float* __restrict__ sp, float* __restrict__ sm,
                                                                 const SgdRanges r, const SgdHyper h,
                                                                 const float* __restrict__ scal) {
    const float lr = scal[0];
    const bool use_m = h.momentum != 0.f;
    float4* p4 = reinterpret_cast<float4*>(p);
    float4* m4 = reinterpret_cast<float4*>(mom);
    float4* sp4 = reinterpret_cast<float4*>(sp);
    float4* sm4 = reinterpret_cast<float4*>(sm);
    const float4 zero = make_float4(0.f, 0.f, 0.f, 0.f);
    const int stride = gridDim.x * kOptThreads;
    for (int q = 0; q < r.nr; ++q) {
        const int hi = r.hi[q];
        for (int i0 = r.lo[q] + blockIdx.x * kOptThreads + threadIdx.x; i0 < hi; i0 += kAheadUnroll * stride) {
            float4 pw[kAheadUnroll], mw[kAheadUnroll];
#pragma unroll
            for (int u = 0; u < kAheadUnroll; ++u) {
                const int i = i0 + u * stride;
                pw[u] = mw[u] = zero;
                if (i < hi) {
                    pw[u] = ld_stream_f4(p4 + i);
                    if (use_m) mw[u] = ld_stream_f4(m4 + i);
                }
            }
#pragma unroll
            for (int u = 0; u < kAheadUnroll; ++u) {
                const int i = i0 + u * stride;
                if (i >= hi) continue;
                st_evict_f4(sp4 + i, pw[u]);
                if (use_m) st_evict_f4(sm4 + i, mw[u]);
                sgd_update4(h, lr, pw[u], zero, mw[u]);
                st_evict_f4(p4 + i, pw[u]);
                if (use_m) st_evict_f4(m4 + i, mw[u]);
            }
        }
    }
}

__device__ __forceinline__ bool any_bits(const float4& v) {
    return (__float_as_uint(v.x) | __float_as_uint(v.y) | __float_as_uint(v.z) | __float_as_uint(v.w)) != 0u;
}

__global__ void __launch_bounds__(kOptThreads) fused_sgd_tail_kernel(float* __restrict__ p, float* __restrict__ g,
                                                                      float* __restrict__ mom,
                                                                      const float* __restrict__ sp,
                                                                      const float* __restrict__ sm, int n,
                                                                      const SgdRanges ahead, const SgdRanges dense,
                                                                      const SgdHyper h, int zero_grad,
                                                                      const float* __restrict__ scal,
                                                                      const int* __restrict__ fault,
                                                                      const int* __restrict__ skip,
                                                                      const float* __restrict__ coef) {
    const bool use_m = h.momentum != 0.f;
    float4* p4 = reinterpret_cast<float4*>(p);
    float4* g4 = reinterpret_cast<float4*>(g);
    float4* m4 = reinterpret_cast<float4*>(mom);
    const float4* sp4 = reinterpret_cast<const float4*>(sp);
    const float4* sm4 = reinterpret_cast<const float4*>(sm);
    const float4 zero = make_float4(0.f, 0.f, 0.f, 0.f);
    const int first = blockIdx.x * kOptThreads + threadIdx.x, stride = gridDim.x * kOptThreads;
    const bool faulted = fault != nullptr && *reinterpret_cast<const volatile int*>(fault) != 0;
    if (faulted || verdict_set(skip)) {
        for (int q = 0; q < ahead.nr; ++q)
            for (int i = ahead.lo[q] + first; i < ahead.hi[q]; i += stride) {
                p4[i] = sp4[i];
                if (use_m) m4[i] = sm4[i];
            }
        if (faulted) return;
        update_pass<1, 1>(p, g, mom, nullptr, n, false, false, zero_grad, scal, nullptr, skip, ClipRef{nullptr, nullptr},
                          [](const float*, float&, float, float&, float&) {});
        return;
    }
    const float lr = scal[0];
    const float c = coef != nullptr ? *coef : 1.f;
    const bool every = c != c;
    for (int q = 0; q < ahead.nr; ++q)
        for (int i = ahead.lo[q] + first; i < ahead.hi[q]; i += stride) {
            float4 gw = ld_stream_f4(g4 + i);
            if (!any_bits(gw) && !every) continue;
            const bool dirty = gw.x != 0.f || gw.y != 0.f || gw.z != 0.f || gw.w != 0.f;
            if (coef != nullptr) scale4(gw, c);
            float4 pw = sp4[i], mw = zero;
            if (use_m) mw = sm4[i];
            sgd_update4(h, lr, pw, gw, mw);
            p4[i] = pw;
            if (use_m) m4[i] = mw;
            if (zero_grad && dirty) g4[i] = zero;
        }
    for (int q = 0; q < dense.nr; ++q)
        for (int i = dense.lo[q] + first; i < dense.hi[q]; i += stride) {
            float4 pw = p4[i], gw = ld_stream_f4(g4 + i), mw = zero;
            const bool dirty = gw.x != 0.f || gw.y != 0.f || gw.z != 0.f || gw.w != 0.f;
            if (coef != nullptr) scale4(gw, c);
            if (use_m && !h.first) mw = m4[i];
            sgd_update4(h, lr, pw, gw, mw);
            p4[i] = pw;
            if (use_m) m4[i] = mw;
            if (zero_grad && dirty) g4[i] = zero;
        }
    if (blockIdx.x == 0)
        for (int i = (n >> 2) * 4 + threadIdx.x; i < n; i += kOptThreads) {
            float pw = p[i], gw = g[i], mw = 0.f;
            if (coef != nullptr) gw = __fmul_rn(gw, c);
            if (use_m && !h.first) mw = mom[i];
            sgd_update(h, lr, pw, gw, mw);
            p[i] = pw;
            if (use_m) mom[i] = mw;
            if (zero_grad) g[i] = 0.f;
        }
}

__global__ void __launch_bounds__(kOptThreads) fused_bert_adam_kernel(float* __restrict__ p, float* __restrict__ g,
                                                                       float* __restrict__ m, float* __restrict__ v,
                                                                       int n, float b1, float b2, float eps, float wd,
                                                                       int zero_grad, const float* __restrict__ scal,
                                                                       const int* __restrict__ fault,
                                                                       const int* __restrict__ skip, const ClipRef clip) {
    update_pass<1, 2>(p, g, m, v, n, true, true, zero_grad, scal, fault, skip, clip,
                      [=](const float* s, float& pw, float gw, float& mw, float& vw) {
                          mw = b1 * mw + (1.f - b1) * gw;
                          vw = b2 * vw + (1.f - b2) * gw * gw;
                          float u = mw / (sqrtf(vw) + eps);
                          if (wd > 0.f) u += wd * pw;
                          pw -= s[0] * u;
                      });
}

__global__ void __launch_bounds__(kOptThreads) fused_adam_kernel(float* __restrict__ p, float* __restrict__ g,
                                                                  float* __restrict__ m, float* __restrict__ v, int n,
                                                                  float w, float b2, float omb2, float eps, float wd,
                                                                  int decoupled, int zero_grad,
                                                                  const float* __restrict__ scal,
                                                                  const int* __restrict__ fault,
                                                                  const int* __restrict__ skip,
                                                                  const float* __restrict__ coef) {
    const bool small_w = fabsf(w) < 0.5f;
    const float lw = small_w ? w : 1.f - w;
    update_pass<3, 2>(p, g, m, v, n, true, true, zero_grad, scal, fault, skip, ClipRef{coef, nullptr},
                      [=](const float* s, float& pw, float gw, float& mw, float& vw) {
                          const float decay = s[0], step_size = s[1], bc2_sqrt = s[2];
                          if (decoupled) pw = pw * decay;
                          else if (wd != 0.f) gw = gw + wd * pw;
                          mw = small_w ? mw + lw * (gw - mw) : gw - (gw - mw) * lw;
                          vw = vw * b2;
                          vw = vw + omb2 * gw * gw;
                          const float d = sqrtf(vw) / bc2_sqrt + eps;
                          pw = pw + (step_size * mw) / d;
                      });
}

__global__ void __launch_bounds__(kOptThreads) momentum_correct_kernel(float* __restrict__ g, float* __restrict__ buf,
                                                                        int n, float momentum) {
    for (int i = blockIdx.x * kOptThreads + threadIdx.x; i < n; i += gridDim.x * kOptThreads) {
        float b = momentum * buf[i] + g[i];
        buf[i] = b;
        g[i] = b;
    }
}

__device__ __forceinline__ double block_sum_d(double v) {
    __shared__ double ws[kOptThreads / 32];
    v = warp_sum_d(v);
    if ((threadIdx.x & 31) == 0) ws[threadIdx.x >> 5] = v;
    __syncthreads();
    double t = 0.0;
    if (threadIdx.x == 0)
        for (int w = 0; w < kOptThreads / 32; ++w) t += ws[w];
    __syncthreads();
    return t;
}

__global__ void __launch_bounds__(kOptThreads) grad_sumsq_kernel(const float* __restrict__ g, const SumsqSegs t,
                                                                  double* __restrict__ partial) {
    int lo = 0, hi = t.nseg - 1;
    while (lo < hi) {
        const int mid = (lo + hi + 1) >> 1;
        if ((int)blockIdx.x >= t.blk_begin[mid]) lo = mid; else hi = mid - 1;
    }
    const int begin = (blockIdx.x - t.blk_begin[lo]) * kSumsqChunk;
    const int len = min(t.len[lo] - begin, kSumsqChunk);
    const float* x = g + t.off[lo] + begin;
    const float4* x4 = reinterpret_cast<const float4*>(x);
    double acc = 0.0;
    for (int i = threadIdx.x; i < (len >> 2); i += kOptThreads) {
        const float4 w = ld_stream_f4(x4 + i);
        acc += (double)w.x * w.x;
        acc += (double)w.y * w.y;
        acc += (double)w.z * w.z;
        acc += (double)w.w * w.w;
    }
    const int i = (len & ~3) + threadIdx.x;
    if (i < len) acc += (double)x[i] * x[i];
    acc = block_sum_d(acc);
    if (threadIdx.x == 0) partial[blockIdx.x] = acc;
}

__global__ void __launch_bounds__(kOptThreads) clip_coef_kernel(const double* __restrict__ partial, int np,
                                                                 const int* __restrict__ seg_blk,
                                                                 const int* __restrict__ seg_scal, int nseg,
                                                                 const float* __restrict__ scal, float max_norm,
                                                                 float* __restrict__ norm, float* __restrict__ coef) {
    if (seg_blk == nullptr) {
        double acc = 0.0;
        for (int i = threadIdx.x; i < np; i += kOptThreads) acc += partial[i];
        acc = block_sum_d(acc);
        if (threadIdx.x == 0) {
            const float nrm = (float)sqrt(acc);
            const float c = __fmul_rn(__frcp_rn(__fadd_rn(nrm, 1e-6f)), max_norm);
            *norm = nrm;
            *coef = c > 1.f ? 1.f : c;
        }
        return;
    }
    const int lane = threadIdx.x & 31;
    for (int s = threadIdx.x >> 5; s < nseg; s += kOptThreads / 32) {
        double acc = 0.0;
        for (int i = seg_blk[s] + lane; i < seg_blk[s + 1]; i += 32) acc += partial[i];
        acc = warp_sum_d(acc);
        if (lane == 0) {
            const float nrm = (float)sqrt(acc);
            const float mx = scal[seg_scal[s]];
            norm[s] = nrm;
            coef[s] = (mx > 0.f && nrm > mx) ? (float)((double)mx / ((double)nrm + 1e-6)) : 1.f;
        }
    }
}

__device__ __forceinline__ float lamb_u(const float* s, float pw, float mw, float vw, float eps) {
    const float mh = __fdiv_rn(mw, s[2]), vh = __fdiv_rn(vw, s[3]);
    return __fmaf_rn(s[1], pw, __fdiv_rn(mh, __fadd_rn(__fsqrt_rn(vh), eps)));
}

__device__ __forceinline__ void lamb_moments(const LambHyper& h, const float* s, float pw, float gw, float& mw,
                                             float& vw, double& aw, double& au) {
    mw = __fmaf_rn(h.omb1, gw, __fmul_rn(h.b1, mw));
    vw = __fmaf_rn(h.omb2, __fmul_rn(gw, gw), __fmul_rn(h.b2, vw));
    const float u = lamb_u(s, pw, mw, vw, h.eps);
    aw += (double)pw * pw;
    au += (double)u * u;
}

__device__ __forceinline__ bool stopped(const int* fault) {
    return fault != nullptr && *reinterpret_cast<const volatile int*>(fault) != 0;
}

__global__ void __launch_bounds__(kOptThreads) lamb_moments_kernel(const float* __restrict__ p, float* __restrict__ g,
                                                                    float* __restrict__ m, float* __restrict__ v,
                                                                    const LambSegs t, const LambHyper h, int zero_grad,
                                                                    const float* __restrict__ scal,
                                                                    const int* __restrict__ fault,
                                                                    const int* __restrict__ skip,
                                                                    const float* __restrict__ coef,
                                                                    double* __restrict__ part_w,
                                                                    double* __restrict__ part_u) {
    if (stopped(fault)) return;
    const int q = __ldg(t.blk) + blockIdx.x;
    int lo = 0, hi = t.nseg - 1;
    while (lo < hi) {
        const int mid = (lo + hi + 1) >> 1;
        if (q >= __ldg(t.blk + mid)) lo = mid; else hi = mid - 1;
    }
    const int begin = (q - __ldg(t.blk + lo)) * kSumsqChunk;
    const int len = min(__ldg(t.len + lo) - begin, kSumsqChunk);
    const int base = __ldg(t.off + lo) + begin;
    const float4* p4 = reinterpret_cast<const float4*>(p + base);
    float4* g4 = reinterpret_cast<float4*>(g + base);
    float4* m4 = reinterpret_cast<float4*>(m + base);
    float4* v4 = reinterpret_cast<float4*>(v + base);
    const float4 zero = make_float4(0.f, 0.f, 0.f, 0.f);
    const int n4 = len >> 2, tail = (len & ~3) + threadIdx.x;
    if (verdict_set(skip)) {
        if (!zero_grad) return;
        for (int i = threadIdx.x; i < n4; i += kOptThreads) {
            const float4 gw = ld_stream_f4(g4 + i);
            if (gw.x != 0.f || gw.y != 0.f || gw.z != 0.f || gw.w != 0.f) g4[i] = zero;
        }
        if (tail < len) g[base + tail] = 0.f;
        return;
    }
    float s[4];
#pragma unroll
    for (int j = 0; j < 4; ++j) s[j] = scal[j];
    const float c = coef != nullptr ? *coef : 1.f;
    double aw = 0.0, au = 0.0;
    for (int i = threadIdx.x; i < n4; i += kOptThreads) {
        const float4 pw = p4[i];
        float4 gw = ld_stream_f4(g4 + i), mw = m4[i], vw = v4[i];
        const bool dirty = gw.x != 0.f || gw.y != 0.f || gw.z != 0.f || gw.w != 0.f;
        if (coef != nullptr) scale4(gw, c);
        lamb_moments(h, s, pw.x, gw.x, mw.x, vw.x, aw, au); lamb_moments(h, s, pw.y, gw.y, mw.y, vw.y, aw, au);
        lamb_moments(h, s, pw.z, gw.z, mw.z, vw.z, aw, au); lamb_moments(h, s, pw.w, gw.w, mw.w, vw.w, aw, au);
        m4[i] = mw;
        v4[i] = vw;
        if (zero_grad && dirty) g4[i] = zero;
    }
    if (tail < len) {
        const int i = base + tail;
        float gw = g[i], mw = m[i], vw = v[i];
        if (coef != nullptr) gw = __fmul_rn(gw, c);
        lamb_moments(h, s, p[i], gw, mw, vw, aw, au);
        m[i] = mw;
        v[i] = vw;
        if (zero_grad) g[i] = 0.f;
    }
    aw = block_sum_d(aw);
    au = block_sum_d(au);
    if (threadIdx.x == 0) {
        part_w[q] = aw;
        part_u[q] = au;
    }
}

__global__ void __launch_bounds__(kOptThreads) lamb_ratio_kernel(const LambSegs t, const double* __restrict__ part_w,
                                                                  const double* __restrict__ part_u,
                                                                  const float* __restrict__ scal,
                                                                  const int* __restrict__ fault,
                                                                  const int* __restrict__ skip,
                                                                  float* __restrict__ norm_w,
                                                                  float* __restrict__ norm_u, float* __restrict__ ratio) {
    if (stopped(fault) || verdict_set(skip)) return;
    const bool decay = scal[1] != 0.f;
    const int lane = threadIdx.x & 31;
    for (int j = threadIdx.x >> 5; j < t.nseg; j += kOptThreads / 32) {
        double aw = 0.0, au = 0.0;
        for (int i = t.blk[j] + lane; i < t.blk[j + 1]; i += 32) {
            aw += part_w[i];
            au += part_u[i];
        }
        aw = warp_sum_d(aw);
        au = warp_sum_d(au);
        if (lane == 0) {
            const double wn = sqrt(aw), un = sqrt(au);
            norm_w[j] = (float)wn;
            norm_u[j] = (float)un;
            ratio[j] = (decay && wn > 0.0 && un > 0.0) ? (float)(wn / un) : 1.f;
        }
    }
}

__global__ void __launch_bounds__(kOptThreads) lamb_apply_kernel(float* __restrict__ p, const float* __restrict__ m,
                                                                  const float* __restrict__ v, int n, float eps,
                                                                  const float* __restrict__ scal,
                                                                  const int* __restrict__ fault,
                                                                  const int* __restrict__ skip, const ClipRef r) {
    if (stopped(fault) || verdict_set(skip)) return;
    float s[4];
#pragma unroll
    for (int j = 0; j < 4; ++j) s[j] = scal[j];
    ClipCursor rc(r);
    const int n4 = n >> 2;
    float4* p4 = reinterpret_cast<float4*>(p);
    const float4* m4 = reinterpret_cast<const float4*>(m);
    const float4* v4 = reinterpret_cast<const float4*>(v);
    for (int i = blockIdx.x * kOptThreads + threadIdx.x; i < n4; i += gridDim.x * kOptThreads) {
        float4 pw = p4[i];
        const float4 mw = ld_stream_f4(m4 + i), vw = ld_stream_f4(v4 + i);
        const float step = __fmul_rn(s[0], rc.at(i));
        pw.x = __fmaf_rn(-step, lamb_u(s, pw.x, mw.x, vw.x, eps), pw.x);
        pw.y = __fmaf_rn(-step, lamb_u(s, pw.y, mw.y, vw.y, eps), pw.y);
        pw.z = __fmaf_rn(-step, lamb_u(s, pw.z, mw.z, vw.z, eps), pw.z);
        pw.w = __fmaf_rn(-step, lamb_u(s, pw.w, mw.w, vw.w, eps), pw.w);
        p4[i] = pw;
    }
    if (blockIdx.x == 0)
        for (int i = n4 * 4 + threadIdx.x; i < n; i += kOptThreads) {
            const float step = __fmul_rn(s[0], rc.at(i >> 2));
            p[i] = __fmaf_rn(-step, lamb_u(s, p[i], m[i], v[i], eps), p[i]);
        }
}

static inline int opt_grid(int n) {
    int g = (n / 4 + kOptThreads - 1) / kOptThreads;
    if (g < 1) g = 1;
    if (g > kStrideGridMax) g = kStrideGridMax;
    return g;
}

cudaError_t launch_fused_sgd(float* p, float* g, float* mom, int n, float momentum, float dampening, float weight_decay,
                             int nesterov, int first_step, int zero_grad, const float* scal, const int* fault,
                             const int* skip, const float* coef, cudaStream_t stream) {
    const SgdHyper h{momentum, dampening, weight_decay, nesterov, first_step};
    fused_sgd_kernel<<<opt_grid(n), kOptThreads, 0, stream>>>(p, g, mom, n, h, zero_grad, scal, fault, skip, coef);
    return cudaGetLastError();
}

cudaError_t launch_sgd_ahead(float* p, float* mom, float* sp, float* sm, const SgdRanges& r, const SgdHyper& h,
                             int max_ctas, const float* scal, cudaStream_t stream) {
    if (h.first) return cudaErrorInvalidValue;
    long long vecs = 0;
    for (int q = 0; q < r.nr; ++q) vecs += r.hi[q] - r.lo[q];
    if (vecs <= 0) return cudaSuccess;
    long long grid = (vecs + kOptThreads * kAheadUnroll - 1) / (kOptThreads * kAheadUnroll);
    grid = std::min<long long>(grid, std::max(max_ctas, 1));
    sgd_ahead_kernel<<<(int)grid, kOptThreads, 0, stream>>>(p, mom, sp, sm, r, h, scal);
    return cudaGetLastError();
}

cudaError_t launch_fused_sgd_tail(float* p, float* g, float* mom, const float* sp, const float* sm, int n,
                                  const SgdRanges& ahead, const SgdRanges& dense, const SgdHyper& h, int zero_grad,
                                  const float* scal, const int* fault, const int* skip, const float* coef,
                                  cudaStream_t stream) {
    fused_sgd_tail_kernel<<<opt_grid(n), kOptThreads, 0, stream>>>(p, g, mom, sp, sm, n, ahead, dense, h, zero_grad,
                                                                  scal, fault, skip, coef);
    return cudaGetLastError();
}

cudaError_t launch_fused_bert_adam(float* p, float* g, float* m, float* v, int n, float b1, float b2, float eps,
                                   float weight_decay, int zero_grad, const float* scal, const int* fault,
                                   const int* skip, const ClipRef& clip, cudaStream_t stream) {
    fused_bert_adam_kernel<<<opt_grid(n), kOptThreads, 0, stream>>>(p, g, m, v, n, b1, b2, eps, weight_decay, zero_grad,
                                                                   scal, fault, skip, clip);
    return cudaGetLastError();
}

cudaError_t launch_fused_adam(float* p, float* g, float* m, float* v, int n, double beta1, double beta2, float eps,
                              float weight_decay, int decoupled, int zero_grad, const float* scal, const int* fault,
                              const int* skip, const float* coef, cudaStream_t stream) {
    fused_adam_kernel<<<opt_grid(n), kOptThreads, 0, stream>>>(p, g, m, v, n, (float)(1.0 - beta1), (float)beta2,
                                                              (float)(1.0 - beta2), eps, weight_decay, decoupled,
                                                              zero_grad, scal, fault, skip, coef);
    return cudaGetLastError();
}

cudaError_t launch_fused_lamb(float* p, float* g, float* m, float* v, int n, double beta1, double beta2, float eps,
                              const LambSegs& t, int nblk, double* part_w, double* part_u, float* norm_w,
                              float* norm_u, float* ratio, int zero_grad, const float* scal, const int* fault,
                              const int* skip, const float* coef, cudaStream_t stream) {
    const LambHyper h{(float)beta1, (float)(1.0 - beta1), (float)beta2, (float)(1.0 - beta2), eps};
    lamb_moments_kernel<<<nblk, kOptThreads, 0, stream>>>(p, g, m, v, t, h, zero_grad, scal, fault, skip, coef, part_w,
                                                          part_u);
    lamb_ratio_kernel<<<1, kOptThreads, 0, stream>>>(t, part_w, part_u, scal, fault, skip, norm_w, norm_u, ratio);
    lamb_apply_kernel<<<opt_grid(n), kOptThreads, 0, stream>>>(p, m, v, n, eps, scal, fault, skip,
                                                               ClipRef{ratio, t.ends});
    return cudaGetLastError();
}

constexpr int kLandThreads = 256;
constexpr int kLandPerCta = 8192;

__global__ void __launch_bounds__(kLandThreads) land_kernel(const LandParams lp, float* __restrict__ bucket) {
    int lo = 0, hi = lp.count - 1;
    while (lo < hi) {
        const int mid = (lo + hi + 1) >> 1;
        if ((int)blockIdx.x >= lp.blk_begin[mid]) lo = mid; else hi = mid - 1;
    }
    const int t = lo;
    const int part = blockIdx.x - lp.blk_begin[t];
    const float* __restrict__ src = lp.src[t];
    float* __restrict__ dst = bucket + lp.dst_off[t];
    const int numel = lp.numel[t];
    const int begin = part * kLandPerCta;
    const int end = min(numel, begin + kLandPerCta);
    if (src == nullptr) {
        for (int i = begin + threadIdx.x; i < end; i += kLandThreads) dst[i] = 0.f;
        return;
    }
    const bool aligned = ((reinterpret_cast<uintptr_t>(src) | reinterpret_cast<uintptr_t>(dst)) & 15u) == 0;
    if (aligned) {
        const int v0 = begin >> 2, v1 = end >> 2;
        const float4* s4 = reinterpret_cast<const float4*>(src);
        float4* d4 = reinterpret_cast<float4*>(dst);
        for (int v = v0 + threadIdx.x; v < v1; v += kLandThreads) st_stream_f4(d4 + v, ld_stream_f4(s4 + v));
        for (int i = (v1 << 2) + threadIdx.x; i < end; i += kLandThreads) dst[i] = src[i];
    } else {
        for (int i = begin + threadIdx.x; i < end; i += kLandThreads) dst[i] = src[i];
    }
}

cudaError_t launch_land(const LandParams& lp, float* bucket, cudaStream_t stream) {
    if (lp.count <= 0) return cudaSuccess;
    land_kernel<<<lp.blk_begin[lp.count], kLandThreads, 0, stream>>>(lp, bucket);
    return cudaGetLastError();
}

cudaError_t launch_momentum_correct(float* g, float* buf, int n, float momentum, cudaStream_t stream) {
    momentum_correct_kernel<<<opt_grid(n), kOptThreads, 0, stream>>>(g, buf, n, momentum);
    return cudaGetLastError();
}

cudaError_t launch_grad_sumsq(const float* g, const SumsqSegs& t, double* partial, cudaStream_t stream) {
    if (t.nseg <= 0) return cudaSuccess;
    grad_sumsq_kernel<<<t.blk_begin[t.nseg], kOptThreads, 0, stream>>>(g, t, partial);
    return cudaGetLastError();
}

cudaError_t launch_clip_coef(const double* partial, int np, const int* seg_blk, const int* seg_scal, int nseg,
                             const float* scal, float max_norm, float* norm, float* coef, cudaStream_t stream) {
    clip_coef_kernel<<<1, kOptThreads, 0, stream>>>(partial, np, seg_blk, seg_scal, nseg, scal, max_norm, norm, coef);
// ... 5 lines not shown
```

oktopk_b200/optimizer.py:

```python
from __future__ import annotations

import math
import os
import warnings
from typing import Dict, Iterable, List, Optional

import torch

from .compression import NoneCompressor, compressors, resolve_compressor
from .config import LossScale, OkTopkConfig
from .ops import ext
from .parallel.allreducer import AllReducer
from .parallel.buckets import Bucket, attach, build_buckets
from .parallel.early_pack import PackPlanner
from .parallel.world import World, world as _world


SGD_AHEAD_CTAS = 24


class _ScaleState:

    def __init__(self, ls: LossScale, device: torch.device):
        self.cfg = ls
        self.buf = torch.zeros(32, dtype=torch.uint8, device=device)
        self.f32 = self.buf[0:8].view(torch.float32)
        self.i32 = self.buf[8:16].view(torch.int32)
        self.i64 = self.buf[16:32].view(torch.int64)
        self.native = device.type == "cuda" and ext.available()
        self.reset()

    @property
    def ptr(self) -> int:
        return self.buf.data_ptr()

    @property
    def found_ptr(self) -> int:
        return self.buf.data_ptr() + 12

    def reset(self, scale: Optional[float] = None, growth_tracker: int = 0, skipped: int = 0, adam_step: int = 0) -> None:
        from .parallel.oracle import inv_scale_of
        scale = self.cfg.init_scale if scale is None else scale
        vals = torch.zeros(32, dtype=torch.uint8)
        vals[0:8].view(torch.float32).copy_(torch.tensor([scale, inv_scale_of(scale)], dtype=torch.float32))
        vals[8:16].view(torch.int32).copy_(torch.tensor([growth_tracker, 0], dtype=torch.int32))
        vals[16:32].view(torch.int64).copy_(torch.tensor([skipped, adam_step], dtype=torch.int64))
        self.buf.copy_(vals)

    def scale(self) -> torch.Tensor:
        return self.f32[0]

    def state(self) -> Dict:
        h = self.buf.cpu()
        f, i, q = h[0:8].view(torch.float32), h[8:16].view(torch.int32), h[16:32].view(torch.int64)
        return {"scale": float(f[0]), "growth_tracker": int(i[0]), "skipped_steps": int(q[0]), "adam_step": int(q[1]),
                "found_inf": int(i[1])}

    def found_host(self) -> bool:
        return bool(self.i32[1].item())

    def check_host(self, flat: torch.Tensor, world: World) -> bool:
        with torch.no_grad():
            bad = (~torch.isfinite(flat)).any().to(torch.int32).reshape(1)
            flat.mul_(self.f32[1])
            world.all_reduce_sum(bad)
            skip = bool(bad.item())
            if skip:
                self.i32[1].fill_(1)
        return skip

    def update(self) -> None:
        c = self.cfg
        if self.native:
            ext.require().scale_update(self.ptr, float(c.growth_factor), float(c.backoff_factor), int(c.growth_interval),
                                       torch.cuda.current_stream().cuda_stream)
            return
        from .parallel.oracle import update_scale
        st = self.state()
        found = bool(st["found_inf"])
        scale, tracker = update_scale(st["scale"], st["growth_tracker"], found, c)
        self.reset(scale, tracker, st["skipped_steps"] + int(found), st["adam_step"] + int(not found))


class _BucketedComm:

    def _okt_setup(self, named_parameters, allreducer: AllReducer, flatten_params: bool = True,
                   loss_scale: Optional[LossScale] = None, max_grad_norm: Optional[float] = None,
                   clip_per_param: bool = False) -> None:
        if named_parameters is not None:
            named_parameters = list(named_parameters)
            if any(not isinstance(p, tuple) for p in named_parameters):
                raise ValueError("named_parameters should be a sequence of (name, parameter) tuples, "
                                 "usually produced by model.named_parameters().")
            names = {v: k for k, v in named_parameters}
        else:
            names = {}
        i = 0
        for g in self.param_groups:
            for p in g["params"]:
                if p not in names:
                    names[p] = "allreduce.noname.%d" % i
                i += 1
        self._parameter_names = names
        self._allreducer = allreducer
        self._cfg: OkTopkConfig = allreducer.cfg
        self.local = False
        self._synced = False
        self._ls: Optional[_ScaleState] = None
        self.momentum_correction = False
        self._buckets: List[Bucket] = build_buckets(self.param_groups, names, self._cfg.bucket_elems)
        self._bucket_of: Dict[torch.nn.Parameter, Bucket] = {}
        self._flat_state: Dict[int, Dict[str, torch.Tensor]] = {}
        self._next_launch = 0
        self._hook_handles = []
        self._comm_stream = None
        self._use_streams = False
        self._land = False
        for b in self._buckets:
            dev = b.params[0].device
            grad = allreducer.register_bucket(b.name, b.numel, dev)
            attach(b, grad, flatten_params)
            if dev.type == "cuda" and self._cfg.land_grads and ext.available():
                self._land = True
            b.pending = len(b.params)
            b.dirty = False
            if dev.type == "cuda":
                self._use_streams = self._cfg.overlap
                b.event = torch.cuda.Event()
            for p in b.params:
                self._bucket_of[p] = b
                self._hook_handles.append(p.register_post_accumulate_grad_hook(self._make_hook(p)))
        if self._update is _AdamUpdate:
            if not (ext.available() and all(b.flat_param is not None and b.grad.is_cuda for b in self._buckets)):
                self._update = None
        self._direct = (self._land and self._update is not None and allreducer.compressor.name == "oktopk"
                        and all(b.flat_param is not None for b in self._buckets))
        self._packs = {}
        self._pos_in_bucket = {p: i for b in self._buckets for i, p in enumerate(b.params)}
        if self._direct and self._use_streams:
            for b in self._buckets:
                if len(b.params) <= ext.require().SRC_SEG_MAX:
                    self._packs[b.index] = PackPlanner(b.offsets, b.numel,
                                                       math.ceil(self._cfg.early_pack_frac * b.numel),
                                                       ext.require().PACK_RANGE_MAX)
            for b in self._buckets:
                b.packing = None
        if self._use_streams:
            self._comm_stream = torch.cuda.Stream(priority=-1)
        self._ahead_stash: Dict[int, tuple] = {}
        self._ahead_stream = None
        self._ahead_ctas = SGD_AHEAD_CTAS
        if (self._packs and self._update is _SGDUpdate and self._cfg.sgd_ahead
                and os.environ.get("OKTOPK_SGD_AHEAD", "1") != "0"):
            self._ahead_stream = torch.cuda.Stream()
            for b in self._buckets:
                if b.index in self._packs:
                    mom = any(self.param_groups[gi].get("momentum", 0.0) != 0 for gi, _, _ in b.group_slices)
                    self._ahead_stash[b.index] = (torch.empty_like(b.grad), torch.empty_like(b.grad) if mom else None)
        for b in self._buckets:
            b.ahead = None
        allreducer.add_resync_hook(self._resync_replicas)
        if loss_scale is not None:
            allreducer.enable_loss_scaling()
            self._ls = _ScaleState(loss_scale, self._buckets[0].params[0].device if self._buckets else torch.device("cpu"))
        self._lr_dev = self._hyper_dev = None
        self._lr_pin, self._lr_ev, self._lr_ring, self._lr_last = [], [], 0, None
        dev0 = self._buckets[0].params[0].device if self._buckets else torch.device("cpu")
        if dev0.type == "cuda" and ext.available() and self._update is not None:
            groups = max(len(self.param_groups), 1)
            self._lr_dev = torch.zeros(groups * self._update.n_scalars, dtype=torch.float32, device=dev0)
            stage = self._lr_dev
            if self._ls is not None and (self._update is _AdamUpdate or self._update is _LambUpdate):
                stage = self._hyper_dev = torch.zeros(groups * 4, dtype=torch.float64, device=dev0)
            self._lr_pin = [torch.zeros_like(stage, device="cpu").pin_memory() for _ in range(8)]
            self._lr_ev = [None] * len(self._lr_pin)
        self._max_grad_norm = max_grad_norm
        self._grad_norm: Optional[torch.Tensor] = None
        self._clip: Optional[_GradClip] = None
        if (max_grad_norm is not None or clip_per_param) and self._device_update():
            self._clip = _GradClip(self, clip_per_param, max_grad_norm or 0.0)
        self._lamb = _LambNorms(self) if self._update is _LambUpdate and self._device_update() else None

    def _resync_replicas(self) -> None:
        w = self._allreducer.world
        if w.size == 1:
            return
        for b in self._buckets:
            if b.flat_param is not None:
                w.broadcast(b.flat_param, 0)
            else:
                for p in b.params:
                    w.broadcast(p.data, 0)
            for t in self._flat_state.get(b.index, {}).values():
                if torch.is_tensor(t):
                    w.broadcast(t, 0)

    @property
    def _okt_adam(self) -> bool:
        return self._update is _AdamUpdate

    def refresh_lr(self) -> None:
        if self._lr_dev is None or self._update is None:
            return
        vals = [self._update.scalars(self, g) for g in self.param_groups]
        if vals == self._lr_last:
            return
        self._lr_ring = (self._lr_ring + 1) % len(self._lr_pin)
        pin = self._lr_pin[self._lr_ring]
        if self._lr_ev[self._lr_ring] is not None:
            self._lr_ev[self._lr_ring].synchronize()
        n = len(vals[0]) if vals else 0
        for gi, sc in enumerate(vals):
            for j, v in enumerate(sc):
                pin[gi * n + j] = v
        (self._hyper_dev if self._hyper_dev is not None else self._lr_dev).copy_(pin, non_blocking=True)
        ev = torch.cuda.Event()
        ev.record()
        self._lr_ev[self._lr_ring] = ev
        self._lr_last = vals

    def _lr_ptr(self, gi: int) -> int:
        return self._lr_dev.data_ptr() + 4 * self._update.n_scalars * gi

    def _maybe_refresh_lr(self) -> None:
        if self._lr_dev is not None and not torch.cuda.is_current_stream_capturing():
            self.refresh_lr()

    def _make_hook(self, p):
        def hook(param):
            b = self._bucket_of[p]
            b.dirty = True
            if self.local:
                return
            b.pending -= 1
            if b.pending == 0:
                self._launch_ready()
            elif b.index in self._packs:
                self._pack_early(b, p)
        return hook

    def _pack_early(self, b: Bucket, p) -> None:
        if b.packing is None:
            b.packing = (self._direct and not self.momentum_correction and self._ls is None
                         and self._allreducer.reads_sources(b.name) and self._allreducer.packs_early(b.name))
        if not b.packing:
            return
        planner = self._packs[b.index]
        ranges = planner.ready(self._pos_in_bucket[p])
        if ranges is None:
            return
        ptrs, offs, lens = [], [], []
        for q, o, v in sorted(zip(b.params, b.offsets, b.grad_views), key=lambda t: t[1]):
            g = q.grad
            if not any(lo <= o < hi for lo, hi in ranges) or g is None or g.numel() == 0:
                continue
            if (g.data_ptr() == v.data_ptr() or g.dtype != torch.float32 or not g.is_cuda or g.stride() != v.stride()
                    or g.data_ptr() % 16):
                raise RuntimeError("early pack: the gradient of %s cannot be read in place; set "
                                   "OkTopkConfig.early_pack=False" % self._parameter_names.get(q, "?"))
            ptrs.append(g.data_ptr())
            offs.append(o)
            lens.append(g.numel())
        if b.ahead is None:
            b.ahead = b.index in self._ahead_stash and self._update.keys[0] in self._flat_state.get(b.index, {})
            if b.ahead:
                self._maybe_refresh_lr()
        ev = torch.cuda.Event()
        ev.record(torch.cuda.current_stream())
        self._comm_stream.wait_event(ev)
        with torch.cuda.stream(self._comm_stream):
            self._allreducer.pack_segment(b.name, ranges, (ptrs, offs, lens), stream=self._comm_stream)
        if b.ahead:
            self._sgd_ahead(b, ranges, ev)

    def _sgd_ahead(self, b: Bucket, ranges, ev) -> None:
        s_ = self._ahead_stream
        if s_ is not self._comm_stream:
            s_.wait_event(ev)
        sp, sm = self._ahead_stash[b.index]
        fs = self._flat_state[b.index]
        C = ext.require()
        for gi, s, e in b.group_slices:
            rs = _clip_ranges(ranges, s, e)
            if not rs:
                continue
            m, damp, wd, nest = _SGDUpdate.hyper(self, self.param_groups[gi])
            C.sgd_ahead(b.flat_param.data_ptr() + 4 * s, fs["momentum_buffer"].data_ptr() + 4 * s, sp.data_ptr() + 4 * s,
                        sm.data_ptr() + 4 * s if sm is not None else 0, e - s, rs, m, damp, wd, int(nest),
                        int(self._ahead_ctas), s_.cuda_stream, self._lr_ptr(gi))

    def _launch_ready(self) -> None:
        while self._next_launch < len(self._buckets) and self._buckets[self._next_launch].pending <= 0:
            self._launch(self._buckets[self._next_launch])
            self._next_launch += 1

    def _land_bucket(self, b: Bucket) -> None:
        srcs, offs, numels = [], [], []
        for p, o, v in zip(b.params, b.offsets, b.grad_views):
            g = p.grad
            if g is None:
                srcs.append(0)
                offs.append(o)
                numels.append(p.numel())
            elif g.data_ptr() == v.data_ptr():
                continue
            elif g.dtype == torch.float32 and g.is_cuda and g.stride() == v.stride():
                srcs.append(g.data_ptr())
                offs.append(o)
                numels.append(g.numel())
            else:
                v.copy_(g)
            p.grad = v
        if srcs:
            ext.require().land_grads(srcs, offs, numels, b.grad.data_ptr(), torch.cuda.current_stream().cuda_stream)

    def _source_table(self, b: Bucket):
        ptrs, offs, lens, held = [], [], [], []
        for p, o, v in zip(b.params, b.offsets, b.grad_views):
            g = p.grad
            if g is None or g.numel() == 0:
                continue
            if (g.data_ptr() == v.data_ptr() or g.dtype != torch.float32 or not g.is_cuda or g.stride() != v.stride()
                    or g.data_ptr() % 16):
                return None
            ptrs.append(g.data_ptr())
            offs.append(o)
            lens.append(g.numel())
            held.append(g)
        if len(ptrs) > ext.require().SRC_SEG_MAX:
            return None
        for p, v in zip(b.params, b.grad_views):
            p.grad = v
# ... 138 lines not shown
    def grad_norm(self) -> Optional[torch.Tensor]:
        return self._grad_norm

    def check_faults(self) -> None:
        self._allreducer.check_faults()

    def close(self) -> None:
        for h in self._hook_handles:
            h.remove()
        self._hook_handles = []
        self._allreducer.close()

    def step(self, closure=None):
        loss = None
        if closure is not None:
            with torch.enable_grad():
                loss = closure()
        if not self.local:
            self.synchronize()
        if self._clip is None and self._max_grad_norm is not None:
            self._grad_norm = torch.nn.utils.clip_grad_norm_([p for g in self.param_groups for p in g["params"]],
                                                             self._max_grad_norm)
        host_skip = self._ls is not None and not self._device_update() and self._ls.found_host()
        if self._update is None:
            if not host_skip:
                super().step()
            for b in self._buckets:
                b.dirty = True
        else:
            self._maybe_refresh_lr()
            if self._hyper_dev is not None:
                ext.require().adam_scalars(self._ls.ptr, self._hyper_dev.data_ptr(), self._lr_dev.data_ptr(),
                                           len(self.param_groups), torch.cuda.current_stream().cuda_stream,
                                           lamb=int(self._update is _LambUpdate))
            if self._clip is not None:
                self._grad_norm = self._clip.run(self)
            with torch.no_grad():
                for b in self._buckets:
                    self._fused_update(b, host_skip)
            self.counter += 1
        if self._ls is not None:
            self._ls.update()
        self._after_step()
        return loss

    def _device_update(self) -> bool:
        return self._update is not None and self._lr_dev is not None and all(
            b.grad.is_cuda and b.flat_param is not None for b in self._buckets)

    def _flat_buffers(self, b: Bucket) -> Dict[str, torch.Tensor]:
        fs = self._flat_state.setdefault(b.index, {})
        for k in self._update.keys:
            if k not in fs:
                fs[k] = torch.zeros_like(b.grad)
                for p, v in zip(b.params, b.views(fs[k])):
                    self.state[p][k] = v
        return fs

    def _fused_update(self, b: Bucket, host_skip: bool = False) -> None:
        first = self._update.keys[0] not in self._flat_state.get(b.index, {})
        fs = self._flat_buffers(b)
        on_gpu = b.grad.is_cuda and b.flat_param is not None and ext.available()
        zero_grad = 0 if self._land and not self._direct else 1
        skip_ptr = self._ls.found_ptr if self._ls is not None else 0
        if b.ahead and on_gpu:
            self._sgd_tail(b, fs, zero_grad, skip_ptr)
            b.dirty = False
            return
        for gi, s, e in b.group_slices:
            def launch(fn, *hyper):
                clip = self._clip.ref(b, s) if self._clip is not None else {}
                fn(b.flat_param.data_ptr() + 4 * s, b.grad.data_ptr() + 4 * s,
                   *(fs[k].data_ptr() + 4 * s for k in self._update.keys), e - s, *hyper, zero_grad,
                   torch.cuda.current_stream().cuda_stream, self._lr_ptr(gi), self._allreducer.fault_ptr(b.name),
                   skip_ptr, **clip)
            if on_gpu or not host_skip:
                self._update.update(self, b, self.param_groups[gi], s, e, fs, first, launch if on_gpu else None)
            if not on_gpu:
                b.grad[s:e].zero_()
        b.dirty = False

    def _sgd_tail(self, b: Bucket, fs: Dict[str, torch.Tensor], zero_grad: int, skip_ptr: int) -> None:
        planner = self._packs[b.index]
        ahead = [r for seg in planner.segments for r in seg]
        rest = planner.rest()
        sp, sm = self._ahead_stash[b.index]
        C = ext.require()
        for gi, s, e in b.group_slices:
            m, damp, wd, nest = _SGDUpdate.hyper(self, self.param_groups[gi])
            C.fused_sgd_tail(b.flat_param.data_ptr() + 4 * s, b.grad.data_ptr() + 4 * s,
                             fs["momentum_buffer"].data_ptr() + 4 * s, sp.data_ptr() + 4 * s,
                             sm.data_ptr() + 4 * s if sm is not None else 0, e - s, _clip_ranges(ahead, s, e),
                             _clip_ranges(rest, s, e), m, damp, wd, int(nest), 0, zero_grad,
                             torch.cuda.current_stream().cuda_stream, self._lr_ptr(gi),
                             self._allreducer.fault_ptr(b.name), skip_ptr,
                             **(self._clip.ref(b, s) if self._clip is not None else {}))

    def _adopt_state(self, counter: Optional[int] = None) -> None:
        keys = self._update.keys
        have = {p for b in self._buckets for p in b.params if self.state.get(p, {}).get(keys[0]) is not None}
        if counter is None:
            steps = {float(self.state[p]["step"]) for p in have if "step" in self.state[p]}
            if len(steps) > 1:
                warnings.warn("DistributedOptimizer: the loaded %s state has unequal step counts per parameter %s; "
                              "using its own step() from now on" % (type(self).__name__, sorted(steps)))
                self._update = None
                self._clip = None
                self._clear_buckets()
                self._direct = False
                for b in self._buckets:
                    for k in keys:
                        self._flat_state.get(b.index, {}).pop(k, None)
                return
            counter = int(steps.pop()) if steps else 0
        self.counter = counter
        loaded = {(p, k): self.state[p][k] for p in have for k in keys}
        with torch.no_grad():
            for b in self._buckets:
                for p in b.params:
                    self.state.get(p, {}).pop("step", None)
                if not any(p in have for p in b.params):
                    for k in keys:
                        self._flat_state.get(b.index, {}).pop(k, None)
                    continue
                fs = self._flat_buffers(b)
                for k in keys:
                    for p, v in zip(b.params, b.views(fs[k])):
                        if p in have:
                            v.copy_(loaded[p, k])
                        else:
                            v.zero_()
                        self.state[p][k] = v


def _clip_ranges(ranges, s: int, e: int):
    top = 4 * ((e - s) // 4)
    out = []
    for lo, hi in ranges:
        lo, hi = max(lo - s, 0), min(hi - s, top)
        if lo < hi:
            out.append((lo, hi))
    return out


class _GradClip:

    def __init__(self, opt, per_param: bool, max_norm: float):
        dev = opt._buckets[0].grad.device
        self.per_param, self.max_norm = per_param, float(max_norm)
        self.segs = None
        if per_param:
            self.segs = _SegTable(opt._buckets, dev)
            self.tables = self.segs.tables
            self.nseg, npart = self.segs.nseg, self.segs.npart
            self.seg_blk, self.ends = self.segs.blk, self.segs.ends
            self.seg_scal = _as_dev([gi * opt._update.n_scalars + 1 for gi in self.segs.group], dev)
        else:
            self.tables = []
            npart = 0
            for b in opt._buckets:
                self.tables.append((b, [0], [b.numel], npart))
                npart += max(1, -(-b.numel // ext.require().SUMSQ_CHUNK))
            self.nseg = 1
            self.seg_blk = self.seg_scal = self.ends = None
        self.partial = torch.zeros(npart, dtype=torch.float64, device=dev)
        self.norm = torch.zeros(self.nseg, dtype=torch.float32, device=dev)
        self.coef = torch.ones(self.nseg, dtype=torch.float32, device=dev)

    def run(self, opt) -> torch.Tensor:
        C, stream = ext.require(), torch.cuda.current_stream().cuda_stream
        for b, offs, lens, p0 in self.tables:
            C.grad_sumsq(b.grad.data_ptr(), offs, lens, self.partial.data_ptr() + 8 * p0, stream)
        if self.per_param:
            C.clip_coef(self.partial.data_ptr(), self.partial.numel(), self.seg_blk.data_ptr(), self.seg_scal.data_ptr(),
                        self.nseg, opt._lr_dev.data_ptr(), 0.0, self.norm.data_ptr(), self.coef.data_ptr(), stream)
            return self.norm
        C.clip_coef(self.partial.data_ptr(), self.partial.numel(), 0, 0, 0, 0, self.max_norm, self.norm.data_ptr(),
                    self.coef.data_ptr(), stream)
        return self.norm[0]
# ... 421 lines not shown
```

oktopk_b200/parallel/allreducer.py:

```python
from __future__ import annotations

import time
from typing import Dict, Optional

import torch

from ..compression import Compressor, resolve_compressor
from ..config import OkTopkConfig
from ..ops import ext
from . import algorithms
from .state import SparseState
from .world import World, world as _world


def _capturing() -> bool:
    return torch.cuda.is_available() and torch.cuda.is_current_stream_capturing()


class AllReducer:
    def __init__(self, compression="oktopk", sparse: bool = True, density: float = 0.01, train_epoch: int = 0,
                 cfg: Optional[OkTopkConfig] = None, world: Optional[World] = None, backend: Optional[str] = None,
                 named_parameters=None, err_callback=None, layerwise_times=None, sigma_scale: float = 2.5,
                 norm_clip: Optional[float] = None, writer=None, **_ignored):
        base = cfg if cfg is not None else OkTopkConfig()
# ... 160 lines not shown
    def save_profiling_norms(self, directory: str, epoch: int) -> None:
        import os
        import numpy as np
        if not self._profiling_norms:
            return
        os.makedirs(directory, exist_ok=True)
        cols = list(zip(*self._profiling_norms))
        for nm, col in zip(("gtopknorm", "randknorm", "upbound", "xnorm", "densestd"), cols):
            np.save(os.path.join(directory, "%s-rank%d-epoch%d.npy" % (nm, self.world.rank, epoch)), np.asarray(col))
        self._profiling_norms = []

    def _reduce_profiled(self, name: str, flat: torch.Tensor, stream, density: float, skip: int = 0) -> torch.Tensor:
        from ..utils.metrics import sparsification_error
        eng = self._engines.get(name)
        st = self._dist_states.get(name)
        res = eng.residual if eng is not None else (st.residual if st is not None else None)
        with torch.no_grad():
            acc = flat.detach().clone()
            if res is not None and res.numel() == acc.numel():
                acc += res
            if self.world.size > 1:
                self.world.all_reduce_sum(acc)
            acc /= self.world.size
        if eng is not None:
            out = eng.reduce(self.compressor.name, density, stream=stream, g=flat, skip=skip)
            if flat.is_cuda:
                torch.cuda.synchronize()
        else:
            if st is None:
                st = self._dist_states[name] = SparseState(flat.numel(), self.world.size)
            out = algorithms.sparse_allreduce(self.compressor.name, flat, st, self.cfg, self.world, density)
        k = max(int(flat.numel() * density), 1)
        rec = sparsification_error(acc, out, k)
        rec["bucket"], rec["density"] = name, density
        self.profile_records.append(rec)
        with torch.no_grad():
            n = acc.numel()
            rk = torch.randperm(n, device=acc.device)[:k]
            randk = torch.zeros_like(acc)
            randk[rk] = acc[rk]
            xnorm = float(acc.norm())
            self._profiling_norms.append((float((acc - out).norm()), float((acc - randk).norm()),
                                          1.0 * (n - k) / n * xnorm, xnorm, float(acc.std())))
        if self.writer is not None and hasattr(self.writer, "add_scalars"):
            self.writer.add_scalars("profiling_norm/" + name, {k2: v for k2, v in rec.items() if isinstance(v, (int, float))},
                                    len(self.profile_records))
        return out

    def run(self, flat_tensor: torch.Tensor, name: str = "flat") -> torch.Tensor:
        assert flat_tensor.dim() == 1 and flat_tensor.dtype == torch.float32
        if name not in self._engines and name not in self._dist_states and self._use_cuda(flat_tensor.device):
            from .gpu_engine import CudaBucketEngine
            self._engines[name] = CudaBucketEngine(flat_tensor.numel(), self.cfg, self.world, name=name)
        return self.reduce_bucket(name, flat_tensor)

    def add_tensor(self, name: str, tensor: torch.Tensor):
        return name

    def get_result(self, name: str):
        raise RuntimeError("results are written in place into the gradient bucket")

    def stop(self) -> None:
        self._running = False

    def stats(self, name: Optional[str] = None) -> Dict:
        out = {}
        for nm, eng in self._engines.items():
            out[nm] = eng.stats()
        for nm, st in self._dist_states.items():
            out[nm] = {"counter": st.counter, "local_thr": st.local_thr, "global_thr": st.global_thr,
                       "local_count": st.last_local_count, "global_count": st.last_global_count,
                       "volume_elems": st.last_volume_elems, "mode": st.last_mode,
                       "edges": st.region_offsets + [st.numel]}
        return out if name is None else out[name]

    def enable_loss_scaling(self) -> None:
        for eng in self._engines.values():
            eng.enable_loss_scaling()

    def fault_ptr(self, name: str) -> int:
        eng = self._engines.get(name)
        return int(eng.fault_ptr) if eng is not None else 0

    def poll_faults(self) -> None:
        if not self._engines:
            return
        if _capturing():
            return
        for eng in self._engines.values():
            if eng.poll_fault():
                self.check_faults()
                return

    def trace(self) -> Dict[str, list]:
        return {nm: eng.trace() for nm, eng in self._engines.items()}

    def resync_hooks(self) -> list:
        return getattr(self, "_resync_hooks", [])

    def add_resync_hook(self, fn) -> None:
        self._resync_hooks = self.resync_hooks() + [fn]

    def check_faults(self) -> None:
        for eng in self._engines.values():
            try:
                eng.check_fault()
            except RuntimeError:
                if self.err_callback is None:
                    raise
                self.err_callback(self.world.size, self.world.rank)
                for e2 in self._engines.values():
                    e2.reset_sparse_state()
                    e2.clear_fault()
                for fn in self.resync_hooks():
                    fn()
                return

    def state_dict(self) -> Dict:
        sd = {"train_epoch": self.train_epoch, "buckets": {}}
        for nm, eng in self._engines.items():
            sd["buckets"][nm] = eng.state_dict()
        for nm, st in self._dist_states.items():
            sd["buckets"][nm] = st.state_dict()
        return sd

    def load_state_dict(self, sd: Dict) -> None:
        self.train_epoch = sd.get("train_epoch", 0)
        for nm, b in sd.get("buckets", {}).items():
            if nm in self._engines:
                self._engines[nm].load_state_dict(b)
            elif nm in self._dist_states:
                dev = self._dist_states[nm].residual.device if self._dist_states[nm].residual is not None else None
                self._dist_states[nm].load_state_dict(b, dev)
            else:
                import warnings
                warnings.warn("checkpoint holds sparse state for bucket %r which is not registered (yet): ignored" % nm)

    def close(self) -> None:
        for eng in self._engines.values():
            eng.close()
        self._engines.clear()


def dense_allreduce(tensor: torch.Tensor, world: Optional[World] = None) -> torch.Tensor:
    return algorithms.dense_allreduce(tensor, world or _world())


def topk_sparse_allreduce(tensor: torch.Tensor, density: float, world: Optional[World] = None, state=None):
    w = world or _world()
    st = state or SparseState(tensor.numel(), w.size)
    return algorithms.topka_allreduce(tensor, st, OkTopkConfig(density=density), w, density)


def gtopk_sparse_allreduce(tensor: torch.Tensor, density: float, world: Optional[World] = None, state=None):
    w = world or _world()
    st = state or SparseState(tensor.numel(), w.size)
    return algorithms.gtopk_allreduce(tensor, st, OkTopkConfig(density=density), w, density)
```

oktopk_b200/parallel/early_pack.py:

```python
from __future__ import annotations

from typing import List, Optional, Sequence, Tuple

Range = Tuple[int, int]


class PackPlanner:

    def __init__(self, offsets: Sequence[int], n: int, min_elems: int, max_ranges: int):
        order = sorted(range(len(offsets)), key=lambda i: offsets[i])
        if any(int(offsets[i]) % 4 for i in order):
            raise ValueError("parameter offsets must be multiples of 4 elements")
        self.n, self.min_elems, self.max_ranges = int(n), max(int(min_elems), 1), int(max_ranges)
        top = 4 * (self.n // 4)
        self._pos = {i: k for k, i in enumerate(order)}
        starts = [min(int(offsets[i]), top) for i in order]
        ends = starts[1:] + [top]
        if starts:
            starts[0] = 0
        self._span = list(zip(starts, ends))
        self.reset()

    def reset(self) -> None:
        self._state = [0] * len(self._span)
        self._pending = 0
        self._segments: List[List[Range]] = []
        self._packed_runs = 0

    @property
    def segments(self) -> List[List[Range]]:
        return [list(s) for s in self._segments]

    def _runs(self, want: int) -> List[Range]:
        out: List[Range] = []
        for (a, b), s in zip(self._span, self._state):
            if s != want or a == b:
                continue
            if out and out[-1][1] == a:
                out[-1] = (out[-1][0], b)
            else:
                out.append((a, b))
        return out

    def ready(self, i: int) -> Optional[List[Range]]:
        k = self._pos[i]
        if self._state[k]:
            return None
        self._state[k] = 1
        self._pending += self._span[k][1] - self._span[k][0]
        if self._pending < self.min_elems:
            return None
        runs = self._runs(1)
        if self._packed_runs + len(runs) > self.max_ranges - 1:
            return None
        for q, s in enumerate(self._state):
            if s == 1:
                self._state[q] = 2
        self._pending = 0
        self._packed_runs += len(runs)
        self._segments.append(runs)
        return runs

    def rest(self) -> List[Range]:
        out: List[Range] = []
        for (a, b), s in zip(self._span, self._state):
            if s == 2 or a == b:
                continue
            if out and out[-1][1] == a:
                out[-1] = (out[-1][0], b)
            else:
                out.append((a, b))
        return out
```

oktopk_b200/parallel/gpu_engine.py:

```python
from __future__ import annotations

import os
from typing import Dict, List, Optional

import torch

from ..config import OkTopkConfig
from ..ops import ext
from .state import CallPlan, SparseState, plan_call, uniform_boundaries, offsets_of
from .symm import SymmBlock, make_symm_block
from .world import World

RES_OKTOPK, RES_LOCAL_GT, RES_LOCAL_GE = 0, 1, 2
GLB_THRESHOLD, GLB_EXACT_TOPK, GLB_ALL_NONZERO = 0, 1, 2
GS_THRESHOLD_REUSE, GS_GAUSSIAN, GS_EXACT_TOPK = 0, 1, 2

_CLASSIC_RESIDUAL = {"topkSA", "topkDSA", "gaussiankSA"}


def _round_up(x: int, m: int) -> int:
    return (int(x) + m - 1) // m * m


class PeerTimeoutError(RuntimeError):
    """A rank of the peer group did not reach a handshake in time (device-side failure detection)."""


class CudaBucketEngine:
    def __init__(self, numel: int, cfg: OkTopkConfig, world: World, name: str = "bucket",
                 max_density: Optional[float] = None, dense_grid: int = 0):
        self.C = ext.require()
        C = self.C
        self.cfg = cfg
        self.world = world
        self.name = name
        self.P = world.size
        self.rank = world.rank
        if self.P > C.MAXP:
            raise ValueError("world size %d exceeds OKT_MAXP=%d" % (self.P, C.MAXP))
        self.n = int(numel)
        self.device = torch.device("cuda", torch.cuda.current_device())
        dmax = max_density if max_density is not None else cfg.density
        if cfg.dynamic_densities:
            dmax = max(dmax, max(cfg.dynamic_densities))
        kmax = max(int(self.n * dmax), 1)
        self.kmax = kmax
        chunk = C.CHUNK
        nmax = _round_up(self.n, chunk)
        if cfg.slot_factor > 0:
            self.cap = min(nmax, _round_up(max(cfg.slot_factor * kmax / self.P, chunk), chunk)) + chunk
        else:
            self.cap = 0
        if cfg.gather_factor > 0 and cfg.compressor not in _CLASSIC_RESIDUAL:
            self.gcap = min(nmax, _round_up(max(cfg.gather_factor * kmax / self.P, 2 * kmax, chunk), chunk)) + chunk
        else:
            self.gcap = nmax + chunk
        info = C.layout_info(self.P, self.n, self.cap, self.gcap)
        self.layout = info
        self.grid = C.max_coop_grid(self.device.index)
        self.gather_grid = C.gather_max_coop_grid(self.device.index)
        self.tree_grid = C.gtopk_max_coop_grid(self.device.index)
        if cfg.comm_ctas > 0:
            self.grid = min(self.grid, cfg.comm_ctas)
            self.gather_grid = min(self.gather_grid, cfg.comm_ctas)
            self.tree_grid = min(self.tree_grid, cfg.comm_ctas)
        sms = torch.cuda.get_device_properties(self.device).multi_processor_count
        self.dense_grid = dense_grid or (min(sms, cfg.comm_ctas) if cfg.comm_ctas > 0 else sms)
        self.grad_bytes = _round_up(self.n * 4, 4096)
        self.comm_off = self.grad_bytes
        self.flags_off = self.comm_off + _round_up(info["total"], 4096)
        flags_bytes = 8 * 2 * self.dense_grid * C.MAXP
        self.block = make_symm_block(self.flags_off + _round_up(flags_bytes, 4096), world, cfg.nvls)
        self.grad = self.block.tensor(0, self.n, "float32")
        self.peer_comm = [p + self.comm_off for p in self.block.ptrs]
        self.peer_grad = [p for p in self.block.ptrs]
        self.peer_flags = [p + self.flags_off for p in self.block.ptrs]
        self.mc_grad = int(getattr(self.block, "mc_ptr", 0) or 0)
        self.state_ptr = C.dev_alloc_zero(C.state_bytes())
        self.fault_ptr = C.fault_ptr(self.state_ptr)
        self.host_flag, self.host_flag_dev = C.host_flag_alloc()
        self.dense_epoch_ptr = C.dev_alloc_zero(8 * self.dense_grid)
        self.scale_sync_ptr = 0
        self.residual = torch.zeros(self.n, dtype=torch.float32, device=self.device)
        if self.cap == 0:
            self.ccap = _round_up(self.n, 32)
        else:
            self.ccap = int(min(_round_up(self.n, 32), max(self.P * self.cap, 32 * kmax + chunk)))
        self.cand = torch.zeros(self.ccap, dtype=torch.int32, device=self.device)
        self._bitmap: Optional[torch.Tensor] = None
        self._sel: Optional[tuple] = None
        self.host = SparseState(self.n, self.P)
        self._write_edges(self.host.region_offsets + [self.n])
        self.last_mode = ""
        self._res_clean = False
        self._skip = 0
        self.early_pack = bool(cfg.early_pack) and os.environ.get("OKTOPK_EARLY_PACK", "1") != "0"

    def _stream(self, stream: Optional[torch.cuda.Stream]) -> int:
        return (stream or torch.cuda.current_stream()).cuda_stream

    def _write_edges(self, edges: List[int], local_thr: float = 0.0, global_thr: float = 0.0) -> None:
        self.C.write_state(self.state_ptr, float(local_thr), float(global_thr), [int(e) for e in edges],
                           torch.cuda.current_stream().cuda_stream)

    def k_now(self, density: Optional[float] = None) -> int:
        d = self.cfg.density if density is None else density
        return max(int(self.n * d), 1)

    def _plan(self, compressor: str, density: Optional[float]) -> CallPlan:
        return plan_call(self.cfg, compressor, self.host.counter, density, self.P)

    def reads_sources(self, compressor: str, density: Optional[float] = None) -> bool:
        return compressor == "oktopk" and self._plan(compressor, density).kind == "fused"

    def packs_early(self, compressor: str, density: Optional[float] = None) -> bool:
        if not (self.early_pack and compressor == "oktopk" and self.cap == 0 and self.cfg.fused):
            return False
        plan = self._plan(compressor, density)
        return plan.kind == "fused" and not plan.exact_local and not plan.repartition

    def pack_segment(self, compressor: str, ranges, srcs: tuple, density: Optional[float] = None,
                     stream: Optional[torch.cuda.Stream] = None) -> None:
        self._fused(compressor, self._plan(compressor, density), density, self._stream(stream), self.grad, srcs,
                    pack_ranges=list(ranges), segment=True)

    def enable_loss_scaling(self) -> None:
        if not self.scale_sync_ptr:
            self.scale_sync_ptr = self.C.dev_alloc_zero(self.C.SCALE_SYNC_BYTES)

    @property
    def verdict_ptr(self) -> int:
        self.enable_loss_scaling()
        return self.scale_sync_ptr + self.C.VERDICT_OFFSET

    def unscale_check(self, loss_scale_ptr: int, stream: Optional[torch.cuda.Stream] = None,
                      srcs: Optional[tuple] = None) -> None:
        self.enable_loss_scaling()
        if srcs is not None and len(srcs[0]):
            ptrs, lens = list(srcs[0]), list(srcs[2])
        else:
            ptrs, lens = [self.grad.data_ptr()], [self.n]
        self.C.unscale_check(ptrs, lens, loss_scale_ptr, self.scale_sync_ptr, self.state_ptr, self.host_flag_dev,
                             self.peer_comm, self.layout["scale_mbox"], self.rank, float(self.cfg.peer_timeout_s),
                             self._stream(stream))

    def reduce(self, compressor: str, density: Optional[float] = None,
               stream: Optional[torch.cuda.Stream] = None, g: Optional[torch.Tensor] = None,
               srcs: Optional[tuple] = None, skip: int = 0, pack_ranges: Optional[list] = None) -> torch.Tensor:
        ext_g = g is not None and g.data_ptr() != self.grad.data_ptr()
        plan = self._plan(compressor, density)
        if srcs is not None and (ext_g or compressor != "oktopk" or plan.kind != "fused"):
            raise ValueError("gradient sources are only read by an Ok-Topk call on the engine's own bucket")
        s = self._stream(stream)
        self._skip = int(skip)
        out = g if ext_g else self.grad
        if plan.kind in ("dense", "dense_switch"):
            if ext_g:
                self.grad.copy_(g)
            if plan.kind == "dense_switch":
                if self._skip:
                    self.C.carry_residual(self.grad.data_ptr(), self.residual.data_ptr(), self.n, self._skip, s)
                elif not self._res_clean:
                    self.grad.add_(self.residual)
                    self.residual.zero_()
                    self._res_clean = True
            self._dense(s)
            if ext_g:
                g.copy_(self.grad)
            self.last_mode = "dense" if plan.kind == "dense" else "dense(auto)"
        else:
            self._res_clean = False
            if plan.kind == "fused":
                self._fused(compressor, plan, density, s, out, srcs, pack_ranges)
            elif plan.kind == "gather":
                self._gather(compressor, plan, density, s, out)
            else:
                self._tree(compressor, density, s, out)
        self.host.counter += 1
        return out

    def _dense(self, s: int) -> None:
        if self.P == 1:
            return
        self.C.dense_run(self.peer_grad, self.peer_flags, self.dense_epoch_ptr, self.n, self.rank,
                         self.dense_grid, s, self.state_ptr, float(self.cfg.peer_timeout_s), self.mc_grad,
                         self.host_flag_dev, self._skip)

    def _fused(self, compressor: str, plan: CallPlan, density: Optional[float], s: int, g: torch.Tensor,
               srcs: Optional[tuple] = None, pack_ranges: Optional[list] = None, segment: bool = False) -> None:
        cfg = self.cfg
        k = self.k_now(density)
        o: Dict = {"pull_tma": 1 if cfg.pull_mode == "tma" else 0, "deterministic": int(cfg.deterministic),
                   "split_phases": 0 if cfg.fused else 1, "timeout_s": float(cfg.peer_timeout_s),
                   "cand": self.cand.data_ptr(), "ccap": self.ccap, "host_fault": self.host_flag_dev,
                   "max_redo": int(cfg.max_redo), "redo_factor": float(cfg.redo_factor),
                   "cand_mode": int(cfg.gselect_mode == "list" or (cfg.gselect_mode == "auto" and k * 200 <= self.n))}
        if compressor == "oktopk":
            o.update(
                exact_local=int(plan.exact_local),
                repartition=int(plan.repartition),
                residual_mode=RES_OKTOPK,
                global_mode=GLB_EXACT_TOPK if plan.exact_global else GLB_THRESHOLD,
                guard_loops=cfg.overselect_guard_loops,
                guard_limit=cfg.overselect_guard_num * k // cfg.overselect_guard_den,
                guard_factor=cfg.overselect_guard_factor,
                cap_limit=int(cfg.overselect_cap * k) if cfg.overselect_cap > 0 else 0,
                cap_rungs=int(cfg.overselect_cap_rungs), cap_factor=float(cfg.overselect_cap_factor),
                l_low_cnt=cfg.local_adapt_low * k, l_high_cnt=cfg.local_adapt_high * k, l_factor=cfg.local_adapt_factor,
                g_low_cnt=cfg.global_adapt_low * k, g_high_cnt=cfg.global_adapt_high * k,
                g_inc=cfg.global_adapt_inc, g_dec=cfg.global_adapt_dec,
            )
        else:
            o.update(exact_local=1, repartition=0,
                     residual_mode=RES_LOCAL_GT if compressor == "gaussiankSA" else RES_LOCAL_GE,
                     global_mode=GLB_ALL_NONZERO, guard_loops=0, guard_limit=0)
            if compressor in ("topkDSA", "topkSA") and g.data_ptr() == self.grad.data_ptr() and self.P > 1 \
                    and cfg.dsa_dense_fallback_frac > 0:
                o["dense_nnz_limit"] = max(int(self.n * cfg.dsa_dense_fallback_frac), 1)
                o["peer_g"] = self.peer_grad
        if srcs is not None:
            o["srcs"] = srcs
        if self._skip:
            o["skip"] = self._skip
        if pack_ranges is not None:
            o["pack_ranges"] = [(int(a), int(b)) for a, b in pack_ranges]
            o["segment"] = int(segment)
            o["seg_ctas"] = int(cfg.early_pack_ctas)
        self.C.oktopk_run(g.data_ptr(), self.residual.data_ptr(), self.state_ptr, self.peer_comm, self.n,
                          self.rank, k, self.cap, self.gcap, o, self.grid, s)
        if not segment:
            self.last_mode = compressor

    def _gather(self, compressor: str, plan: CallPlan, density: Optional[float], s: int, g: torch.Tensor) -> None:
        cfg = self.cfg
        d = cfg.density if density is None else density
        k = self.k_now(density)
        o: Dict = {"density": d, "pull_tma": 1 if cfg.pull_mode == "tma" else 0, "timeout_s": float(cfg.peer_timeout_s),
                   "host_fault": self.host_flag_dev}
        if cfg.norm_clip is not None and compressor in ("topkA", "topkA2"):
            o["clip_max_norm"] = float((1.0 / self.P) ** 0.5 * cfg.norm_clip)
        if compressor in ("topkA", "topkA2"):
            o["select_mode"] = GS_EXACT_TOPK
            if compressor == "topkA2":
                o.update(reselect=1, bitmap=self._bitmap_ptr(), cand=self.cand.data_ptr(), ccap=self.ccap)
        elif compressor == "topkAopt":
            o["select_mode"] = GS_THRESHOLD_REUSE
            o["exact_now"] = int(plan.exact_local)
        else:
            o["select_mode"] = GS_GAUSSIAN
            o["gauss_mode"] = {"vgg": 0, "lstm": 1, "bert": 2}[cfg.gaussian_mode]
            o["gauss_loops"] = cfg.gaussian_loops
            o["gauss_factor"] = cfg.gaussian_factor
        if self._skip:
            o["skip"] = self._skip
        self.C.gather_run(g.data_ptr(), self.residual.data_ptr(), self.state_ptr, self.peer_comm, self.n,
                          self.rank, k, self.cap, self.gcap, o, self.gather_grid, s)
        self.last_mode = compressor

    def _bitmap_ptr(self) -> int:
        if self._bitmap is None:
            self._bitmap = torch.zeros((self.n + 31) // 32 + 32, dtype=torch.int32, device=self.device)
        return self._bitmap.data_ptr()

    def _tree(self, compressor: str, density: Optional[float], s: int, g: torch.Tensor) -> None:
        cfg = self.cfg
        k = self.k_now(density)
        if self._sel is None:
            selcap = int(min(_round_up(self.n, 32), 2 * self.kmax + self.C.CHUNK))
            self._sel = (torch.zeros(selcap, dtype=torch.int32, device=self.device),
                         torch.zeros(selcap, dtype=torch.float32, device=self.device), selcap)
        o: Dict = {"pull_tma": 1 if cfg.pull_mode == "tma" else 0, "timeout_s": float(cfg.peer_timeout_s),
                   "host_fault": self.host_flag_dev, "bitmap": self._bitmap_ptr(), "cand": self.cand.data_ptr(),
                   "ccap": self.ccap, "sel_idx": self._sel[0].data_ptr(), "sel_val": self._sel[1].data_ptr(),
                   "selcap": self._sel[2]}
        if cfg.norm_clip is not None:
            o["clip_max_norm"] = float((1.0 / self.P) ** 0.5 * cfg.norm_clip)
        if self._skip:
# ... 79 lines not shown
```

Before: 14850.

## Record global top-k indices for a sparse SGD tail and add late ahead-updates

During the final gather, the top-k kernel now writes the indices it keeps into a fix-up list with a count and an overflow flag. The fused SGD tail uses this list to update only those elements in already-updated ranges, replacing a full scan of the gradient over those ranges. The Python planner also launches extra 'late' ahead-SGD updates for parameters that become ready after the first pack, shrinking the dense tail. The cost is atomics on the gather path, an atomicExch per element, and more bookkeeping, with a fallback to the full scan when the list overflows.

```diff
diff --git a/oktopk_b200/csrc/bindings.cpp b/oktopk_b200/csrc/bindings.cpp
--- a/oktopk_b200/csrc/bindings.cpp
+++ b/oktopk_b200/csrc/bindings.cpp
@@ -203,6 +203,7 @@
     d["cum_overflow_send"] = s->cum_overflow_send; d["cum_overflow_gather"] = s->cum_overflow_gather;
     d["cum_redo"] = s->cum_redo;
     d["fault"] = s->fault;
+    d["fix_count"] = s->fix_count; d["fix_over"] = s->fix_over;
     auto us = [&](int a, int b) { return s->t_phase[b] >= s->t_phase[a] ? (double)(s->t_phase[b] - s->t_phase[a]) * 1e-3 : 0.0; };
     py::dict ph;
     ph["local"] = us(5, 0); ph["pack"] = us(0, 1); ph["wait_rs"] = us(1, 6); ph["reduce"] = us(6, 2); ph["gselect"] = us(2, 3);
@@ -272,6 +273,11 @@
     if (!o.contains("cand") || !o.contains("ccap")) throw std::runtime_error("oktopk_run: candidate scratch missing");
     p.cand = P_<int>(o["cand"].cast<uint64_t>()); p.ccap = o["ccap"].cast<int>();
     p.cand_mode = o.contains("cand_mode") ? o["cand_mode"].cast<int>() : 1;
+    if (o.contains("fix")) {
+        p.fix = P_<int>(o["fix"].cast<uint64_t>());
+        p.fix_cap = o["fix_cap"].cast<int>();
+        if (p.fix == nullptr || p.fix_cap <= 0) throw std::runtime_error("oktopk_run: the fix-up list needs a capacity");
+    }
     fill_peers(p.peers, peers);
     p.P = (int)peers.size(); p.rank = rank; p.n = n; p.k = k;
     p.L = make_layout(p.P, n, cap, gcap);
@@ -505,14 +511,18 @@
                            const std::vector<std::pair<long long, long long>>& ahead,
                            const std::vector<std::pair<long long, long long>>& dense, double momentum, double dampening,
                            double wd, int nesterov, int first, int zero_grad, uint64_t stream, uint64_t scal_ptr,
-                           uint64_t fault_ptr, uint64_t skip_ptr, uint64_t coef_ptr) {
+                           uint64_t fault_ptr, uint64_t skip_ptr, uint64_t coef_ptr, uint64_t fix_ptr,
+                           uint64_t fix_count_ptr, int fix_cap, long long fix_base) {
     if (scal_ptr == 0) throw std::runtime_error("fused_sgd_tail: scal_ptr must point at the group's device scalars");
     if (momentum != 0.0 && (mom == 0 || sm == 0)) throw std::runtime_error("fused_sgd_tail: momentum needs mom and sm");
+    if (fix_ptr != 0 && (fix_count_ptr == 0 || fix_cap <= 0 || fix_base < 0))
+        throw std::runtime_error("fused_sgd_tail: a fix-up list needs its count word, a capacity and the slice start");
     const SgdHyper h{(float)momentum, (float)dampening, (float)wd, nesterov, first};
+    const SgdFix fix{P_<const int>(fix_ptr), P_<const int>(fix_count_ptr), fix_cap, (int)fix_base};
     ck(launch_fused_sgd_tail(P_<float>(p), P_<float>(g), P_<float>(mom), P_<const float>(sp), P_<const float>(sm), n,
                              sgd_ranges(ahead, n, "fused_sgd_tail"), sgd_ranges(dense, n, "fused_sgd_tail"), h,
                              zero_grad, P_<float>(scal_ptr), P_<int>(fault_ptr), P_<int>(skip_ptr),
-                             P_<const float>(coef_ptr), S_(stream)),
+                             P_<const float>(coef_ptr), fix, S_(stream)),
        "fused_sgd_tail");
 }
 static void fused_bert_adam(uint64_t p, uint64_t g, uint64_t m, uint64_t v, int n, double b1, double b2, double eps,
@@ -940,6 +950,7 @@
     m.def("host_flag_read", &host_flag_read);
     m.def("host_flag_clear", &host_flag_clear);
     m.def("fault_ptr", [](uint64_t st) { return (uint64_t)&P_<OktState>(st)->fault; });
+    m.def("fix_count_ptr", [](uint64_t st) { return (uint64_t)&P_<OktState>(st)->fix_count; });
     m.def("gather_max_coop_grid", &gather_max_coop_grid);
     m.def("gtopk_max_coop_grid", &gtopk_max_coop_grid);
     m.def("vmm_probe", &vmm_probe);
@@ -966,7 +977,8 @@
     m.def("fused_sgd_tail", &fused_sgd_tail, py::arg("p"), py::arg("g"), py::arg("mom"), py::arg("sp"), py::arg("sm"),
           py::arg("n"), py::arg("ahead"), py::arg("dense"), py::arg("momentum"), py::arg("dampening"), py::arg("wd"),
           py::arg("nesterov"), py::arg("first"), py::arg("zero_grad"), py::arg("stream"), py::arg("scal_ptr"),
-          py::arg("fault_ptr") = 0, py::arg("skip_ptr") = 0, py::arg("coef_ptr") = 0);
+          py::arg("fault_ptr") = 0, py::arg("skip_ptr") = 0, py::arg("coef_ptr") = 0, py::arg("fix_ptr") = 0,
+          py::arg("fix_count_ptr") = 0, py::arg("fix_cap") = 0, py::arg("fix_base") = 0);
     m.def("fused_bert_adam", &fused_bert_adam, py::arg("p"), py::arg("g"), py::arg("m"), py::arg("v"), py::arg("n"),
           py::arg("b1"), py::arg("b2"), py::arg("eps"), py::arg("wd"), py::arg("zero_grad"), py::arg("stream"),
           py::arg("scal_ptr"), py::arg("fault_ptr") = 0, py::arg("skip_ptr") = 0, py::arg("coef_ptr") = 0,
diff --git a/oktopk_b200/csrc/oktopk.cu b/oktopk_b200/csrc/oktopk.cu
--- a/oktopk_b200/csrc/oktopk.cu
+++ b/oktopk_b200/csrc/oktopk.cu
@@ -306,6 +306,8 @@
     const float thr_in = st->local_thr;
     const bool exact_local = p.exact_local || thr_in == 0.f;
     const bool two_pass = exact_local || p.repartition;
+    const bool records_fix = p.fix != nullptr && !two_pass && p.residual_mode == RES_OKTOPK &&
+                             p.global_mode != GLB_ALL_NONZERO;
     uint32_t pipe_it = 0;
 
     for (int b = tid; b < kHistBins; b += kThreads) s_hist[b] = 0;
@@ -637,6 +639,8 @@
                 st->pack_thr = thr_sel;
                 st->stat_local_count = cnt;
                 st->tie_cursor = 0;
+                st->fix_count = 0;
+                st->fix_over = records_fix ? 0 : 1;
                 float nt = t;
                 if ((double)cnt < p.l_low_cnt) nt = t / p.l_factor;
                 else if ((double)cnt > p.l_high_cnt) nt = t * p.l_factor;
@@ -874,8 +878,14 @@
             __syncthreads();
             const bool exact = p.global_mode == GLB_EXACT_TOPK;
             pull_chunks(s_srcs, P, p.pull_tma != 0, &s_pull, pipe_it, [&](int sl, int idx, float val) {
-                if ((unsigned)idx >= (unsigned)n) return;
-                bool keep = exact ? (fabsf(val) >= gsel) : true;
+                const bool keep = (unsigned)idx < (unsigned)n && (exact ? (fabsf(val) >= gsel) : true);
+                if (records_fix) {
+                    const int pos = warp_append_active(&st->fix_count, keep);
+                    if (keep) {
+                        if (pos < p.fix_cap) p.fix[pos] = idx;
+                        else st->fix_over = 1;
+                    }
+                }
                 if (!keep) return;
                 kept_cnt++;
                 p.g[idx] = val / fP;
diff --git a/oktopk_b200/csrc/oktopk.cuh b/oktopk_b200/csrc/oktopk.cuh
--- a/oktopk_b200/csrc/oktopk.cuh
+++ b/oktopk_b200/csrc/oktopk.cuh
@@ -47,6 +47,8 @@
     uint32_t sel_prefix;
     uint32_t sel_krem;
     int tie_cursor;
+    int fix_count;
+    int fix_over;
     int cuts[OKT_MAXP];
     int stat_local_count;
     int stat_global_count;
@@ -176,6 +178,8 @@
     int pk_mode, pk_nr;
     int pk_lo[kPackRangeMax];
     int pk_hi[kPackRangeMax];
+    int* fix;
+    int fix_cap;
 };
 static_assert(sizeof(OktParams) <= 4096, "OktParams must fit the 4 KB kernel-parameter limit");
 
@@ -276,10 +280,15 @@
 };
 cudaError_t launch_sgd_ahead(float* p, float* mom, float* sp, float* sm, const SgdRanges& r, const SgdHyper& h,
                              int max_ctas, const float* scal, cudaStream_t stream);
+struct SgdFix {
+    const int* idx;
+    const int* count;
+    int cap, base;
+};
 cudaError_t launch_fused_sgd_tail(float* p, float* g, float* mom, const float* sp, const float* sm, int n,
                                   const SgdRanges& ahead, const SgdRanges& dense, const SgdHyper& h, int zero_grad,
                                   const float* scal, const int* fault, const int* skip, const float* coef,
-                                  cudaStream_t stream);
+                                  const SgdFix& fix, cudaStream_t stream);
 cudaError_t launch_fused_bert_adam(float* p, float* g, float* m, float* v, int n, float b1, float b2, float eps,
                                    float weight_decay, int zero_grad, const float* scal, const int* fault,
                                    const int* skip, const ClipRef& clip, cudaStream_t stream);
diff --git a/oktopk_b200/csrc/optim.cu b/oktopk_b200/csrc/optim.cu
--- a/oktopk_b200/csrc/optim.cu
+++ b/oktopk_b200/csrc/optim.cu
@@ -23,6 +23,10 @@
 
 __device__ __forceinline__ void scale4(float4& gw, float c) {
     gw.x = __fmul_rn(gw.x, c); gw.y = __fmul_rn(gw.y, c); gw.z = __fmul_rn(gw.z, c); gw.w = __fmul_rn(gw.w, c);
+}
+
+__device__ __forceinline__ bool any_bits(const float4& v) {
+    return (__float_as_uint(v.x) | __float_as_uint(v.y) | __float_as_uint(v.z) | __float_as_uint(v.w)) != 0u;
 }
 
 template <int kScal, int kState, typename Upd>
@@ -40,8 +44,7 @@
     if (verdict_set(skip)) {
         if (!zero_grad) return;
         for (int i = blockIdx.x * kOptThreads + threadIdx.x; i < n4; i += gridDim.x * kOptThreads) {
-            const float4 gw = ld_stream_f4(g4 + i);
-            if (gw.x != 0.f || gw.y != 0.f || gw.z != 0.f || gw.w != 0.f) g4[i] = zero;
+            if (any_bits(ld_stream_f4(g4 + i))) g4[i] = zero;
         }
         if (blockIdx.x == 0)
             for (int i = n4 * 4 + threadIdx.x; i < n; i += kOptThreads) g[i] = 0.f;
@@ -53,7 +56,7 @@
     ClipCursor cc(clip);
     for (int i = blockIdx.x * kOptThreads + threadIdx.x; i < n4; i += gridDim.x * kOptThreads) {
         float4 pw = p4[i], gw = ld_stream_f4(g4 + i), mw = zero, vw = zero;
-        const bool dirty = gw.x != 0.f || gw.y != 0.f || gw.z != 0.f || gw.w != 0.f;
+        const bool dirty = any_bits(gw);
         if (clip.coef != nullptr) scale4(gw, cc.at(i));
         if (load) {
             mw = m4[i];
@@ -157,10 +160,6 @@
     }
 }
 
-__device__ __forceinline__ bool any_bits(const float4& v) {
-    return (__float_as_uint(v.x) | __float_as_uint(v.y) | __float_as_uint(v.z) | __float_as_uint(v.w)) != 0u;
-}
-
 __global__ void __launch_bounds__(kOptThreads) fused_sgd_tail_kernel(float* __restrict__ p, float* __restrict__ g,
                                                                       float* __restrict__ mom,
                                                                       const float* __restrict__ sp,
@@ -170,7 +169,7 @@
                                                                       const float* __restrict__ scal,
                                                                       const int* __restrict__ fault,
                                                                       const int* __restrict__ skip,
-                                                                      const float* __restrict__ coef) {
+                                                                      const float* __restrict__ coef, const SgdFix fix) {
     const bool use_m = h.momentum != 0.f;
     float4* p4 = reinterpret_cast<float4*>(p);
     float4* g4 = reinterpret_cast<float4*>(g);
@@ -194,23 +193,47 @@
     const float lr = scal[0];
     const float c = coef != nullptr ? *coef : 1.f;
     const bool every = c != c;
-    for (int q = 0; q < ahead.nr; ++q)
-        for (int i = ahead.lo[q] + first; i < ahead.hi[q]; i += stride) {
-            float4 gw = ld_stream_f4(g4 + i);
-            if (!any_bits(gw) && !every) continue;
-            const bool dirty = gw.x != 0.f || gw.y != 0.f || gw.z != 0.f || gw.w != 0.f;
-            if (coef != nullptr) scale4(gw, c);
-            float4 pw = sp4[i], mw = zero;
-            if (use_m) mw = sm4[i];
-            sgd_update4(h, lr, pw, gw, mw);
-            p4[i] = pw;
-            if (use_m) m4[i] = mw;
-            if (zero_grad && dirty) g4[i] = zero;
-        }
+    if (every || fix.idx == nullptr || fix.count[1] != 0) {
+        for (int q = 0; q < ahead.nr; ++q)
+            for (int i = ahead.lo[q] + first; i < ahead.hi[q]; i += stride) {
+                float4 gw = ld_stream_f4(g4 + i);
+                const bool dirty = any_bits(gw);
+                if (!dirty && !every) continue;
+                if (coef != nullptr) scale4(gw, c);
+                float4 pw = sp4[i], mw = zero;
+                if (use_m) mw = sm4[i];
+                sgd_update4(h, lr, pw, gw, mw);
+                p4[i] = pw;
+                if (use_m) m4[i] = mw;
+                if (zero_grad && dirty) g4[i] = zero;
+            }
+    } else {
+        const int cnt = min(fix.count[0], fix.cap);
+        for (int e = first; e < cnt; e += stride) {
+            const int i = fix.idx[e] - fix.base, v = i >> 2;
+            if (i < 0 || i >= n) continue;
+            bool in = false;
+            for (int q = 0; q < ahead.nr; ++q) in |= v >= ahead.lo[q] && v < ahead.hi[q];
+            if (!in) continue;
+            float gw;
+            if (zero_grad) {
+                gw = atomicExch(g + i, 0.f);
+                if (__float_as_uint(gw) == 0u) continue;
+            } else {
+                gw = g[i];
+            }
+            float pw = sp[i], mw = 0.f;
+            if (coef != nullptr) gw = __fmul_rn(gw, c);
+            if (use_m) mw = sm[i];
+            sgd_update(h, lr, pw, gw, mw);
+            p[i] = pw;
+            if (use_m) mom[i] = mw;
+        }
+    }
     for (int q = 0; q < dense.nr; ++q)
         for (int i = dense.lo[q] + first; i < dense.hi[q]; i += stride) {
             float4 pw = p4[i], gw = ld_stream_f4(g4 + i), mw = zero;
-            const bool dirty = gw.x != 0.f || gw.y != 0.f || gw.z != 0.f || gw.w != 0.f;
+            const bool dirty = any_bits(gw);
             if (coef != nullptr) scale4(gw, c);
             if (use_m && !h.first) mw = m4[i];
             sgd_update4(h, lr, pw, gw, mw);
@@ -229,6 +252,7 @@
             if (zero_grad) g[i] = 0.f;
         }
 }
+
 
 __global__ void __launch_bounds__(kOptThreads) fused_bert_adam_kernel(float* __restrict__ p, float* __restrict__ g,
                                                                        float* __restrict__ m, float* __restrict__ v,
@@ -392,8 +416,7 @@
     if (verdict_set(skip)) {
         if (!zero_grad) return;
         for (int i = threadIdx.x; i < n4; i += kOptThreads) {
-            const float4 gw = ld_stream_f4(g4 + i);
-            if (gw.x != 0.f || gw.y != 0.f || gw.z != 0.f || gw.w != 0.f) g4[i] = zero;
+            if (any_bits(ld_stream_f4(g4 + i))) g4[i] = zero;
         }
         if (tail < len) g[base + tail] = 0.f;
         return;
@@ -406,7 +429,7 @@
     for (int i = threadIdx.x; i < n4; i += kOptThreads) {
         const float4 pw = p4[i];
         float4 gw = ld_stream_f4(g4 + i), mw = m4[i], vw = v4[i];
-        const bool dirty = gw.x != 0.f || gw.y != 0.f || gw.z != 0.f || gw.w != 0.f;
+        const bool dirty = any_bits(gw);
         if (coef != nullptr) scale4(gw, c);
         lamb_moments(h, s, pw.x, gw.x, mw.x, vw.x, aw, au); lamb_moments(h, s, pw.y, gw.y, mw.y, vw.y, aw, au);
         lamb_moments(h, s, pw.z, gw.z, mw.z, vw.z, aw, au); lamb_moments(h, s, pw.w, gw.w, mw.w, vw.w, aw, au);
@@ -519,11 +542,12 @@
 cudaError_t launch_fused_sgd_tail(float* p, float* g, float* mom, const float* sp, const float* sm, int n,
                                   const SgdRanges& ahead, const SgdRanges& dense, const SgdHyper& h, int zero_grad,
                                   const float* scal, const int* fault, const int* skip, const float* coef,
-                                  cudaStream_t stream) {
+                                  const SgdFix& fix, cudaStream_t stream) {
     fused_sgd_tail_kernel<<<opt_grid(n), kOptThreads, 0, stream>>>(p, g, mom, sp, sm, n, ahead, dense, h, zero_grad,
-                                                                  scal, fault, skip, coef);
-    return cudaGetLastError();
-}
+                                                                  scal, fault, skip, coef, fix);
+    return cudaGetLastError();
+}
+
 
 cudaError_t launch_fused_bert_adam(float* p, float* g, float* m, float* v, int n, float b1, float b2, float eps,
                                    float weight_decay, int zero_grad, const float* scal, const int* fault,
diff --git a/oktopk_b200/optimizer.py b/oktopk_b200/optimizer.py
--- a/oktopk_b200/optimizer.py
+++ b/oktopk_b200/optimizer.py
@@ -17,6 +17,8 @@
 
 
 SGD_AHEAD_CTAS = 24
+
+SGD_AHEAD_LATE_FRAC = 0.09
 
 
 class _ScaleState:
@@ -155,6 +157,7 @@
             self._ahead_stream = torch.cuda.Stream()
             for b in self._buckets:
                 if b.index in self._packs:
+                    self._packs[b.index].ahead_min = max(math.ceil(SGD_AHEAD_LATE_FRAC * b.numel), 1)
                     mom = any(self.param_groups[gi].get("momentum", 0.0) != 0 for gi, _, _ in b.group_slices)
                     self._ahead_stash[b.index] = (torch.empty_like(b.grad), torch.empty_like(b.grad) if mom else None)
         for b in self._buckets:
@@ -248,6 +251,12 @@
         planner = self._packs[b.index]
         ranges = planner.ready(self._pos_in_bucket[p])
         if ranges is None:
+            if b.ahead:
+                late = planner.late()
+                if late is not None:
+                    ev = torch.cuda.Event()
+                    ev.record(torch.cuda.current_stream())
+                    self._sgd_ahead(b, late, ev)
             return
         ptrs, offs, lens = [], [], []
         for q, o, v in sorted(zip(b.params, b.offsets, b.grad_views), key=lambda t: t[1]):
@@ -552,19 +561,21 @@
 
     def _sgd_tail(self, b: Bucket, fs: Dict[str, torch.Tensor], zero_grad: int, skip_ptr: int) -> None:
         planner = self._packs[b.index]
-        ahead = [r for seg in planner.segments for r in seg]
-        rest = planner.rest()
+        ahead = planner.updated()
+        rest = planner.not_updated()
         sp, sm = self._ahead_stash[b.index]
         C = ext.require()
+        stream = torch.cuda.current_stream().cuda_stream
+        fault = self._allreducer.fault_ptr(b.name)
+        fix = self._allreducer.fix_list(b.name)
         for gi, s, e in b.group_slices:
             m, damp, wd, nest = _SGDUpdate.hyper(self, self.param_groups[gi])
             C.fused_sgd_tail(b.flat_param.data_ptr() + 4 * s, b.grad.data_ptr() + 4 * s,
                              fs["momentum_buffer"].data_ptr() + 4 * s, sp.data_ptr() + 4 * s,
                              sm.data_ptr() + 4 * s if sm is not None else 0, e - s, _clip_ranges(ahead, s, e),
-                             _clip_ranges(rest, s, e), m, damp, wd, int(nest), 0, zero_grad,
-                             torch.cuda.current_stream().cuda_stream, self._lr_ptr(gi),
-                             self._allreducer.fault_ptr(b.name), skip_ptr,
-                             **(self._clip.ref(b, s) if self._clip is not None else {}))
+                             _clip_ranges(rest, s, e), m, damp, wd, int(nest), 0, zero_grad, stream, self._lr_ptr(gi),
+                             fault, skip_ptr, **(self._clip.ref(b, s) if self._clip is not None else {}),
+                             **(dict(fix, fix_base=s) if fix is not None else {}))
 
     def _adopt_state(self, counter: Optional[int] = None) -> None:
         keys = self._update.keys
diff --git a/oktopk_b200/parallel/allreducer.py b/oktopk_b200/parallel/allreducer.py
--- a/oktopk_b200/parallel/allreducer.py
+++ b/oktopk_b200/parallel/allreducer.py
@@ -266,6 +266,12 @@
         eng = self._engines.get(name)
         return int(eng.fault_ptr) if eng is not None else 0
 
+    def fix_list(self, name: str) -> Optional[dict]:
+        eng = self._engines.get(name)
+        if eng is None:
+            return None
+        return {"fix_ptr": eng.fix.data_ptr(), "fix_count_ptr": int(eng.fix_count_ptr), "fix_cap": eng.fix_cap}
+
     def poll_faults(self) -> None:
         if not self._engines:
             return
diff --git a/oktopk_b200/parallel/early_pack.py b/oktopk_b200/parallel/early_pack.py
--- a/oktopk_b200/parallel/early_pack.py
+++ b/oktopk_b200/parallel/early_pack.py
@@ -7,11 +7,13 @@
 
 class PackPlanner:
 
-    def __init__(self, offsets: Sequence[int], n: int, min_elems: int, max_ranges: int):
+    def __init__(self, offsets: Sequence[int], n: int, min_elems: int, max_ranges: int,
+                 ahead_min: Optional[int] = None):
         order = sorted(range(len(offsets)), key=lambda i: offsets[i])
         if any(int(offsets[i]) % 4 for i in order):
             raise ValueError("parameter offsets must be multiples of 4 elements")
         self.n, self.min_elems, self.max_ranges = int(n), max(int(min_elems), 1), int(max_ranges)
+        self.ahead_min = None if ahead_min is None else max(int(ahead_min), 1)
         top = 4 * (self.n // 4)
         self._pos = {i: k for k, i in enumerate(order)}
         starts = [min(int(offsets[i]), top) for i in order]
@@ -24,6 +26,7 @@
     def reset(self) -> None:
         self._state = [0] * len(self._span)
         self._pending = 0
+        self._late_pending = 0
         self._segments: List[List[Range]] = []
         self._packed_runs = 0
 
@@ -31,10 +34,10 @@
     def segments(self) -> List[List[Range]]:
         return [list(s) for s in self._segments]
 
-    def _runs(self, want: int) -> List[Range]:
+    def _runs(self, *want: int) -> List[Range]:
         out: List[Range] = []
         for (a, b), s in zip(self._span, self._state):
-            if s != want or a == b:
+            if s not in want or a == b:
                 continue
             if out and out[-1][1] == a:
                 out[-1] = (out[-1][0], b)
@@ -48,6 +51,8 @@
             return None
         self._state[k] = 1
         self._pending += self._span[k][1] - self._span[k][0]
+        if self._segments:
+            self._late_pending += self._span[k][1] - self._span[k][0]
         if self._pending < self.min_elems:
             return None
         runs = self._runs(1)
@@ -57,9 +62,30 @@
             if s == 1:
                 self._state[q] = 2
         self._pending = 0
+        self._late_pending = 0
         self._packed_runs += len(runs)
         self._segments.append(runs)
         return runs
+
+    def late(self) -> Optional[List[Range]]:
+        if self.ahead_min is None or not self._segments or self._late_pending < self.ahead_min:
+            return None
+        runs = self._runs(1)
+        marked = [q for q, s in enumerate(self._state) if s == 1]
+        for q in marked:
+            self._state[q] = 3
+        if len(self._runs(2, 3)) > self.max_ranges - 1:
+            for q in marked:
+                self._state[q] = 1
+            return None
+        self._late_pending = 0
+        return runs
+
+    def updated(self) -> List[Range]:
+        return self._runs(2, 3)
+
+    def not_updated(self) -> List[Range]:
+        return self._runs(0, 1)
 
     def rest(self) -> List[Range]:
         out: List[Range] = []
diff --git a/oktopk_b200/parallel/gpu_engine.py b/oktopk_b200/parallel/gpu_engine.py
--- a/oktopk_b200/parallel/gpu_engine.py
+++ b/oktopk_b200/parallel/gpu_engine.py
@@ -87,6 +87,9 @@
         else:
             self.ccap = int(min(_round_up(self.n, 32), max(self.P * self.cap, 32 * kmax + chunk)))
         self.cand = torch.zeros(self.ccap, dtype=torch.int32, device=self.device)
+        self.fix_cap = int(min(_round_up(self.n, 32), 4 * kmax + chunk))
+        self.fix = torch.zeros(self.fix_cap, dtype=torch.int32, device=self.device)
+        self.fix_count_ptr = C.fix_count_ptr(self.state_ptr)
         self._bitmap: Optional[torch.Tensor] = None
         self._sel: Optional[tuple] = None
         self.host = SparseState(self.n, self.P)
@@ -193,6 +196,7 @@
         o: Dict = {"pull_tma": 1 if cfg.pull_mode == "tma" else 0, "deterministic": int(cfg.deterministic),
                    "split_phases": 0 if cfg.fused else 1, "timeout_s": float(cfg.peer_timeout_s),
                    "cand": self.cand.data_ptr(), "ccap": self.ccap, "host_fault": self.host_flag_dev,
+                   "fix": self.fix.data_ptr(), "fix_cap": self.fix_cap,
                    "max_redo": int(cfg.max_redo), "redo_factor": float(cfg.redo_factor),
                    "cand_mode": int(cfg.gselect_mode == "list" or (cfg.gselect_mode == "auto" and k * 200 <= self.n))}
         if compressor == "oktopk":
```

Result: faster. 15170 (median of 6 runs) (+2.1%).
